# laprade117/interactive-unet

Hardware: AMD Instinct MI355X
Metric: voxels/sec (train step + full-volume predict) on 128^3 chunks (higher is better)
Workload: dtype bf16

## Files before the change

### include/iunet.h

```cpp
#ifndef IUNET_H
#define IUNET_H
#ifdef __cplusplus
extern "C" {
#endif

const char* iunet_last_error(void);
int iunet_abi_version(void);

long long iunet_pack_conv3_elems(int Cout, int Cin, int taps, int mode);
int iunet_pack_conv3(int dtype, const void* w, const void* scale, void* dst, int Cout, int Cin, int taps, int mode,
                     void* stream);
long long iunet_pack_first_conv_elems(int Cout, int Cin, int taps);
int iunet_pack_first_conv(int dtype, const void* w, const void* scale, void* dst, int Cout, int Cin, int taps,
                          void* stream);
int iunet_pack_convT(int dtype, const void* w, void* dst, int Cin, int Cout, int npos, void* stream);

int iunet_pack_desc_bytes(void);
int iunet_pack_batch(const void* descs, int n, int quant_max_cout, void* stream);

int iunet_conv3_fwd(int dtype, int nd, const void* x, long long x_sstride, void* y, long long y_sstride,
                    const void* wpk, const void* bias, void* stats, int N, int D, int H, int W, int Cin, int Cout,
                    int epi, int layout, void* stream);
int iunet_conv3_pick_layout(int nd, int N, int D, int H, int W, int Cin, int Cout);
int iunet_conv3_tile_pairs(int nd, int N, int D, int H, int W, int Cin, int Cout);
// ... 43 lines not shown
                            const void* weight, int tdtype, int kind, void* slab, void* out4, void* coef, int N, long long vox,
                            void* stream);
int iunet_f32_head_loss_bwd(const void* x, long long x_ss, int C0, const void* w, const void* bias, int ncls, const void* target,
                            const void* weight, int tdtype, const void* coef, void* dlogits, long long dl_ss, void* dx, long long dx_ss,
                            int N, long long vox, void* stream);
int iunet_f32_channel_sum(const void* t, long long t_ss, void* out, int C, int N, long long vox, void* stream);

int iunet_x2_convT_kc(int Cin);
int iunet_x2_prep(const void* w, void* wv, void* oscale, void* bias_out, const void* gamma, const void* beta, const void* mean,
                  const void* var, const void* bias_in, float eps, float act_in, float act_out, int Cout, int Cin, int taps,
                  int transposed, int chunk, void* stream);
int iunet_x2_prep_desc_bytes(void);
int iunet_x2_prep_batch(const void* table, int n, int rows, void* stream);
int iunet_x2m_prep_batch(const void* table, int n, int rows, void* stream);
int iunet_x2_first_conv_fwd(int nd, const void* x, int in_dtype, const long long* in_strides, void* y, long long y_sstride, int y_lo,
                            const void* w, const void* oscale, const void* bias, float act_scale, int N, int D, int H, int W, int Cin,
                            int Cout, int relu, void* stream);
int iunet_x2_pack_mode(int nd);
int iunet_x2_conv3_fwd(int nd, const void* x, long long x_sstride, int x_lo, void* y, long long y_sstride, int y_lo, const void* wpk,
                       const void* oscale, const void* bias, int N, int D, int H, int W, int Cin, int Cout, int epi, void* stream);
int iunet_x2_conv3_fwd_flag(int nd, const void* x, long long x_sstride, int x_lo, void* y, long long y_sstride, int y_lo, const void* wpk,
                            const void* oscale, const void* bias, int N, int D, int H, int W, int Cin, int Cout, int epi, void* sat, void* stream);
int iunet_x2_maxpool_fwd(int nd, const void* x, long long x_ss, int x_lo, void* y, long long y_ss, int y_lo, int C, int N, int Do,
                         int Ho, int Wo, void* stream);
int iunet_x2_convT_fwd(int nd, const void* x, long long x_ss, int x_lo, void* y, long long y_ss, int y_lo, const void* wpk,
                       const void* oscale, const void* bias, int N, int D, int H, int W, int Cin, int Cout, void* stream);
int iunet_x2_head_fwd(const void* x, long long x_ss, int x_lo, int C0, const void* w, const void* bias, float act_scale, int ncls,
                      void* logits, void* probs, void* cls, const long long* out_strides, float divisor, int accumulate, int N, int D,
                      int H, int W, void* stream);

long long iunet_x2m_w8_bytes(int Cout, int Cin);
int iunet_x2m_prep(const void* w, void* whi, void* w8, void* oscale, void* bias_out, const void* gamma, const void* beta, const void* mean,
                   const void* var, float eps, float act_in, float act_out, int Cout, int Cin, void* stream);
long long iunet_x2m_w8_bytes_nd(int nd, int Cout, int Cin);
int iunet_x2m_prep_nd(int nd, const void* w, void* whi, void* w8, void* oscale, void* bias_out, const void* gamma, const void* beta,
                      const void* mean, const void* var, float eps, float act_in, float act_out, int Cout, int Cin, void* stream);
int iunet_x2m_conv_fwd(int nd, const void* x, long long x_ss, const void* x8, long long x8_ss, void* y, long long y_ss, int y_lo, void* y8,
                       long long y8_ss, const void* w16, const void* w8, const void* oscale, const void* bias, int N, int D, int H, int W,
                       int Cin, int Cout, int epi, void* sat, void* stream);
int iunet_x2m_pool_fusable(int nd, int C);
int iunet_x2m_conv_pool_fwd(int nd, const void* x, long long x_ss, const void* x8, long long x8_ss, void* y, long long y_ss, int y_lo, void* y8,
                            long long y8_ss, void* py, long long py_ss, void* py8, long long py8_ss, const void* w16, const void* w8,
                            const void* oscale, const void* bias, int N, int D, int H, int W, int Cin, int Cout, int epi, void* sat, void* stream);
int iunet_x2m_first_stage_fusable(int nd, int cin, int c0, int N, int H, int W);
int iunet_x2m_first_stage_fwd(const void* x, int in_dtype, const long long* in_strides, const void* fw, const void* f_oscale, const void* f_bias,
                              float act_scale, void* y, long long y_ss, int y_lo, void* y8, long long y8_ss, void* py, long long py_ss, void* py8,
                              long long py8_ss, const void* w16, const void* w8, const void* oscale, const void* bias, int N, int H, int W,
                              void* sat, void* stream);
int iunet_x2m_head_fusable(int ncls, int C0);
int iunet_x2m_conv_head_fwd(int nd, const void* x, long long x_ss, const void* x8, long long x8_ss, const void* w16, const void* w8,
                            const void* oscale, const void* bias, const void* head_w, const void* head_b, float act_scale, int ncls,
                            void* logits, void* probs, void* cls, const long long* out_strides, float divisor, int accumulate, int N, int D,
                            int H, int W, int Cin, void* sat, void* stream);
int iunet_x2m_make8(const void* x, long long x_ss, int x_lo, void* x8, long long x8_ss, int C, int N, int D, int H, int W, void* stream);
int iunet_x2m_first_conv_fwd(int nd, const void* x, int in_dtype, const long long* in_strides, void* y, long long y_sstride, int y_lo,
                             void* y8, long long y8_sstride, const void* w, const void* oscale, const void* bias, float act_scale, int N,
                             int D, int H, int W, int Cin, int Cout, int relu, void* sat, void* stream);
int iunet_x2m_convT_fwd(int nd, const void* x, long long x_ss, int x_lo, void* y, long long y_ss, int y_lo, void* y8, long long y8_ss,
                        const void* wpk, const void* oscale, const void* bias, int N, int D, int H, int W, int Cin, int Cout, void* sat, void* stream);
int iunet_x2m_maxpool_fwd(int nd, const void* x, long long x_ss, const void* x8, long long x8_ss, void* y, long long y_ss, void* y8,
                          long long y8_ss, int C, int N, int Do, int Ho, int Wo, void* stream);
int iunet_x2m_conv3_fwd(const void* x, long long x_ss, const void* x8, long long x8_ss, void* y, long long y_ss, int y_lo, void* y8,
                        long long y8_ss, const void* w16, const void* w8, const void* oscale, const void* bias, int N, int D, int H, int W,
                        int Cin, int Cout, int epi, void* sat, void* stream);

typedef struct iunet_net iunet_net;
int iunet_net_create(int dim, int levels, int base, int cin, int ncls, int mode, float act_scale, iunet_net** out);
int iunet_net_create_ex(int dim, int levels, int base, int cin, int ncls, int mode, float act_scale, int norm, int groups, iunet_net** out);
int iunet_net_create_nested(int dim, int levels, int base, int cin, int ncls, int mode, iunet_net** out);
void iunet_net_destroy(iunet_net* net);
long long iunet_net_num_params(const iunet_net* net);
int iunet_net_num_tensors(const iunet_net* net);
int iunet_net_param(const iunet_net* net, int index, char* name, int name_cap, long long* offset, long long* numel);
long long iunet_net_packed_bytes(const iunet_net* net);
int iunet_net_load(iunet_net* net, const void* flat_params, void* packed, void* stream);
long long iunet_net_workspace_bytes(const iunet_net* net, int N, int D, int H, int W);
int iunet_net_forward(iunet_net* net, const void* x, int in_dtype, const long long* in_strides, int N, int D, int H, int W, void* workspace,
                      void* logits, void* probs, void* cls, const long long* out_strides, float divisor, int accumulate, void* stream);
int iunet_net_forward_argmax(iunet_net* net, const void* x_u8, void* cls_u8, int N, int D, int H, int W, void* workspace, void* stream);
long long iunet_net_eval_scratch_bytes(const iunet_net* net, int N, int D, int H, int W);
int iunet_net_eval_step(iunet_net* net, const void* x, int in_dtype, const long long* in_strides, const void* target, const void* weight,
                        int tdtype, int loss_kind, int N, int D, int H, int W, void* workspace, void* scratch, void* out4, void* stream);

int iunet_f8_pack_order(int taps, int Cin);
long long iunet_f8_pack_conv3_bytes(int Cout, int Cin, int taps);
int iunet_f8_pack_conv3(const void* w, const void* gamma, const void* beta, const void* mean, const void* var, float eps,
                        void* dst, void* wscale, void* bias_out, int Cout, int Cin, int taps, void* stream);
long long iunet_conv3_f8_workspace_elems(int nd, int N, int D, int H, int W, int Cin, int Cout);
int iunet_conv3_f8_fwd(int dtype, int nd, const void* x, long long x_sstride, void* y, long long y_sstride, const void* wpk,
                       const void* wscale, const void* bias, int N, int D, int H, int W, int Cin, int Cout, int epi,
                       void* workspace, void* stream);
int iunet_conv3_f8_fwd_q(int dtype, int nd, const void* x, long long x_sstride, int x_fmt, void* y, long long y_sstride, int y_fmt,
                         const void* wpk, const void* wscale, const void* bias, int N, int D, int H, int W, int Cin, int Cout, int epi,
                         void* workspace, void* stream);
int iunet_first_conv_fwd_q(int dtype, int nd, const void* x, int in_dtype, const long long* in_strides, void* y,
                           long long y_sstride_bytes, const void* w, const void* bias, int N, int D, int H, int W,
                           int Cin, int Cout, int relu, void* stream);
int iunet_maxpool_q_fwd(int nd, const void* x, long long x_ss_bytes, void* y, long long y_ss_bytes, int C, int N, int Do, int Ho, int Wo,
                        void* stream);
int iunet_convT_fwd_q(int dtype, int nd, const void* x, long long x_ss, void* y, long long y_ss_bytes, const void* wpk,
                      const void* bias, int N, int D, int H, int W, int Cin, int Cout, void* stream);

long long iunet_gn_precise_slab_bytes(int N, int C, long long vox);
int iunet_f32_gn_relu_fwd(const void* x, long long x_ss, void* y, long long y_ss, const void* gamma, const void* beta, int groups, float eps,
                          void* slab, void* scale, void* shift, int C, int N, long long vox, void* stream);
int iunet_x2_gn_relu_fwd(const void* x, long long x_ss, int x_lo, void* y, long long y_ss, int y_lo, const void* gamma, const void* beta,
// ... 202 lines not shown
```

### interactive-unet_amd/csrc/conv3_x2m.hip

```cpp
#include "common.h"
#include "x2_prep_desc.h"
#ifdef X2M_ABLATE_NO_MFMA
template <typename A, typename B> __device__ __forceinline__ f32x4 x2m_ablate(const A a, const B b, f32x4 c) {
  c[0] = fmaf(__builtin_bit_cast(float, (unsigned)__builtin_bit_cast(unsigned long long, *(const unsigned long long*)&a)),
              __builtin_bit_cast(float, (unsigned)__builtin_bit_cast(unsigned long long, *(const unsigned long long*)&b)), c[0]);
  return c;
}
#define X2M_MFMA16(a, b, c) x2m_ablate(a, b, c)
#define X2M_MFMA128(a, b, c) x2m_ablate(a, b, c)
#define X2M_MFMA32F8(a, b, c) x2m_ablate(a, b, c)
#else
#define X2M_MFMA16(a, b, c) __builtin_amdgcn_mfma_f32_16x16x32_f16(a, b, c, 0, 0, 0)
#define X2M_MFMA128(a, b, c) __builtin_amdgcn_mfma_scale_f32_16x16x128_f8f6f4(a, b, c, 0, 0, 0, 0, 0, 0)
#define X2M_MFMA32F8(a, b, c) __builtin_amdgcn_mfma_f32_16x16x32_fp8_fp8(a, b, c, 0, 0, 0)
#endif
#include <cstdlib>
#include <type_traits>

namespace {

typedef long i64;
typedef int i32x8 __attribute__((ext_vector_type(8)));
typedef u32x2_t u32x2;

// ... 33 lines not shown
  f16x8 hi;
#pragma unroll
  for (int c = 0; c < NCLS; ++c) l[c] = 0.f;
#pragma unroll
  for (int j = 0; j < 8; ++j) {
    const float v = fminf(fmaxf(r[j], -65504.f), 65504.f);
    const f16 h = (f16)v;
    const f16 lw = (f16)(v - (float)h);
    hi[j] = h;
    const float a = ((float)h + (float)lw) * p.inv_act;
#pragma unroll
    for (int c = 0; c < NCLS; ++c) l[c] = fmaf(a, hw[c * 32 + q * 8 + j], l[c]);
  }
  if (ok && p.sat != nullptr) x2_note_saturation(p.sat, hi);
#pragma unroll
  for (int c = 0; c < NCLS; ++c) {
    l[c] = __fadd_rn(l[c], __shfl_xor(l[c], 16));
    l[c] = __fadd_rn(l[c], __shfl_xor(l[c], 32));
    l[c] = __fadd_rn(l[c], hw[NCLS * 32 + c]);
  }
}
template <int NCLS>
__device__ __forceinline__ void x2m_head_store(const ConvX2MParams& p, const float (&l)[NCLS], bool ok, int n_img, long long nvox, long long vo,
                                               int gz, int gy, int gx) {
  if (!ok) return;
  const long long obase = n_img * p.oN + gz * p.oD + gy * p.oH + gx * p.oW;
  float mx = l[0];
#pragma unroll
  for (int c = 1; c < NCLS; ++c) mx = fmaxf(mx, l[c]);
  if (p.logits) {
#pragma unroll
    for (int c = 0; c < NCLS; ++c) p.logits[obase + c * p.oC] = l[c];
  }
  float e[NCLS], sum = 0.f;
#pragma unroll
  for (int c = 0; c < NCLS; ++c) { e[c] = expf(l[c] - mx); sum += e[c]; }
  float pr[NCLS];
  pr[0] = __fdiv_rn(e[0], sum);
  float pm = pr[0]; int am = 0;
#pragma unroll
  for (int c = 1; c < NCLS; ++c) { pr[c] = __fdiv_rn(e[c], sum); if (pr[c] > pm) { pm = pr[c]; am = c; } }
  if (p.cls) p.cls[n_img * nvox + vo] = (unsigned char)am;
  if (p.probs) {
#pragma unroll
    for (int c = 0; c < NCLS; ++c) {
      float* o = p.probs + obase + c * p.oC;
      float rr = p.accumulate ? __fadd_rn(*o, pr[c]) : pr[c];
      if (p.divisor != 1.0f) rr = __fdiv_rn(rr, p.divisor);
      *o = rr;
    }
  }
}

template <bool SMALL, int HEAD = 0, bool POOL = false>
__global__ __launch_bounds__((XMTile<SMALL>::NCW * 64 + XM_NLT), 1) void conv3_x2m_kernel(ConvX2MParams p) {
  static_assert(!(POOL && HEAD > 0), "the pooled conv is an encoder conv: no head");
  using TL = XMTile<SMALL>;
  constexpr int NCW = TL::NCW, NLT = XM_NLT, NLW = NLT / 64;
  constexpr int TZ = TL::TZ, TY = TL::TY, TX = TL::TX;
  constexpr int NI = TZ * TY / NCW, NR = NI;
  constexpr int PZ = TZ + 2, PY = TY + 2, PX = TX + 2;
  constexpr int NPIX = PZ * PY * PX;
  constexpr int PLANE16 = ((NPIX * 16 + 255) / 256) * 256;
  constexpr int A16 = 2 * PLANE16;
  constexpr int NCMB = 5, W16 = NCMB * 3 * 2 * 1024;
  constexpr int ZS = 192;
  constexpr int PLANE8 = PZ * ZS * 16;
  constexpr int A8 = 2 * PLANE8;
  constexpr int W128 = 2 * 3 * 2 * 2 * 1024, W32 = 3 * 2 * 512, W8 = W128 + W32;
  constexpr int OFF_A16 = 0, OFF_W16 = A16, OFF_A8 = OFF_W16 + W16, OFF_W8 = OFF_A8 + A8, OFF_E = OFF_W8 + W8;
  constexpr int OFF_P = OFF_E + 256;
  static_assert(NI == 4 && NCW * NI == TZ * TY, "a consumer wave owns 4 rows of one z slice");

  extern __shared__ __attribute__((aligned(256))) unsigned char smem[];

  const int tid = threadIdx.x, lane = tid & 63;
  const int wave = __builtin_amdgcn_readfirstlane(tid >> 6);
  const int cob = blockIdx.y;
  const int nbricks = p.N * p.nbz * p.nby * p.nbx;
  const int xcd = (blockIdx.x + (nbricks < 8 ? blockIdx.y : 0)) & 7, slot = blockIdx.x >> 3;
  const int sx = slot % p.bx, sy = (slot / p.bx) % p.by, sz = slot / (p.bx * p.by);
  const int b_begin = (int)((long long)xcd * nbricks / 8), b_end = (int)((long long)(xcd + 1) * nbricks / 8);
  const int nchunk = p.Cin / 16;
  const int npairs = (b_end - b_begin) * nchunk;
  if (npairs <= 0) return;
  const long long plane_stride = (long long)p.D * p.H * p.W * 8;
  const long long plane16b = (long long)p.D * p.H * p.W * 16;

  auto tile_origin = [&](int k, int& n_img, int& z0, int& y0, int& x0) -> bool {
    int b = b_begin + k;
    const int Bx = b % p.nbx; b /= p.nbx;
    const int By = b % p.nby; b /= p.nby;
    const int Bz = b % p.nbz; n_img = b / p.nbz;
    const int tz = Bz * p.bz + sz, ty = By * p.by + sy, tx = Bx * p.bx + sx;
    z0 = tz * TZ; y0 = ty * TY; x0 = tx * TX;
    return tz < p.tilesZ && ty < p.tilesY && tx < p.tilesX;
  };
  const unsigned lds0 = (unsigned)(size_t)(__attribute__((address_space(3))) unsigned char*)smem;
  if (tid < 64) ((float*)(smem + OFF_E))[tid] = tid < 32 ? p.oscale[cob * 32 + tid] : (p.epi != 0 ? p.bias[cob * 32 + tid - 32] : 0.f);
  if constexpr (HEAD > 0) {
    for (int i = tid; i < HEAD * 33; i += (int)blockDim.x) ((float*)(smem + OFF_E + 256))[i] = i < HEAD * 32 ? p.head_w[i] : p.head_b[i - HEAD * 32];
  }

  if (wave >= NCW) {
    const unsigned* zero16 = iunet_opaque_ptr((const unsigned*)g_xm_zero16);
    const int lt = tid - NCW * 64;
    const int lw = __builtin_amdgcn_readfirstlane(lt >> 6);
    auto dma_piece = [&](const unsigned char* gsrc, unsigned dst) {
      unsigned keep;
      asm volatile("s_mov_b32 %0, m0\n\ts_mov_b32 m0, %2\n\ts_nop 0\n\tglobal_load_lds_dwordx4 %1, off\n\ts_mov_b32 m0, %0"
                   : "=&s"(keep) : "v"(gsrc), "s"(dst) : "memory");
    };
    auto dma_weights = [&](const unsigned char* ws, int off, int bytes) {
      const int npiece = bytes / 1024;
      for (int piece = lw; piece < npiece; piece += NLW)
        dma_piece(ws + piece * 1024 + (lt & 63) * 16, __builtin_amdgcn_readfirstlane(lds0 + off + piece * 1024));
    };
    constexpr int AIT = (PLANE16 / 16 + NLT - 1) / NLT;
    int pcoord[AIT];
#pragma unroll
    for (int it = 0; it < AIT; ++it) {
      const int pix = min(lt + it * NLT, NPIX - 1);
      const int px = pix % PX, t2 = pix / PX;
      pcoord[it] = px | ((t2 % PY) << 8) | ((t2 / PY) << 16);
    }
    constexpr int NSLOT = PZ * ZS;
    constexpr int DIT = (NSLOT + NLT - 1) / NLT;
    static_assert(NSLOT % 64 == 0, "an e4m3 plane is whole wave instructions");
    int dcoord[DIT];
#pragma unroll
    for (int it = 0; it < DIT; ++it) {
      const int s = lt + it * NLT;
      const int pz = s / ZS, rem = s - pz * ZS, py = rem / PX, px = rem - py * PX;
      dcoord[it] = (s < NSLOT && rem < PY * PX) ? (px | (py << 8) | (pz << 16)) : -1;
    }
    auto dma16 = [&](int k) {
      const int tile = k / nchunk, chunk = k - tile * nchunk;
      int n_img, z0, y0, x0;
      tile_origin(tile, n_img, z0, y0, x0);
      dma_weights((const unsigned char*)p.w16 + ((long long)cob * nchunk + chunk) * W16, OFF_W16, W16);
      const f16* xc = (const f16*)p.x + (long long)n_img * p.x_sstride + (long long)chunk * 2 * plane_stride;
#pragma unroll
      for (int it = 0; it < AIT; ++it) {
        const int base = it * NLT + lw * 64;
        if (base < PLANE16 / 16) {
          const int pix = lt + it * NLT;
          const int px = pcoord[it] & 255, py = (pcoord[it] >> 8) & 255, pz = pcoord[it] >> 16;
          const int gz = z0 + pz - 1, gy = y0 + py - 1, gx = x0 + px - 1;
          const bool ok = pix < NPIX && (unsigned)gz < (unsigned)p.D && (unsigned)gy < (unsigned)p.H && (unsigned)gx < (unsigned)p.W;
          const long long goff = (((long long)gz * p.H + gy) * p.W + gx) * 8;
          if (pix < PLANE16 / 16) {
#pragma unroll
            for (int e = 0; e < 2; ++e)
              dma_piece(ok ? (const unsigned char*)(xc + e * plane_stride + goff) : (const unsigned char*)zero16,
                        __builtin_amdgcn_readfirstlane(lds0 + OFF_A16 + e * PLANE16 + base * 16));
          }
        }
      }
    };
    auto dma8 = [&](int k) {
      const int tile = k / nchunk, chunk = k - tile * nchunk;
      int n_img, z0, y0, x0;
      tile_origin(tile, n_img, z0, y0, x0);
      dma_weights((const unsigned char*)p.w8 + ((long long)cob * nchunk + chunk) * W8, OFF_W8, W8);
      const unsigned char* xc = (const unsigned char*)p.x8 + (long long)n_img * p.x8_sstride + (long long)chunk * plane16b;
#pragma unroll
      for (int it = 0; it < DIT; ++it) {
        const int base = it * NLT + lw * 64;
        if (base < NSLOT) {
          const int c = dcoord[it];
          const int gz = z0 + (c >> 16) - 1, gy = y0 + ((c >> 8) & 255) - 1, gx = x0 + (c & 255) - 1;
          const bool ok = c >= 0 && (unsigned)gz < (unsigned)p.D && (unsigned)gy < (unsigned)p.H && (unsigned)gx < (unsigned)p.W;
          const long long goff = (((long long)gz * p.H + gy) * p.W + gx) * 16;
          dma_piece(ok ? xc + goff : (const unsigned char*)zero16, __builtin_amdgcn_readfirstlane(lds0 + OFF_A8 + base * 16));
        }
      }
    };
    auto make_hi8 = [&]() {
      f16x8 va[DIT], vb[DIT];
#pragma unroll
      for (int it = 0; it < DIT; ++it) {
        const int c = dcoord[it];
        const int pix = c >= 0 ? ((c >> 16) * PY + ((c >> 8) & 255)) * PX + (c & 255) : 0;
        va[it] = *(const f16x8*)(smem + OFF_A16 + pix * 16);
        vb[it] = *(const f16x8*)(smem + OFF_A16 + PLANE16 + pix * 16);
      }
#pragma unroll
      for (int it = 0; it < DIT; ++it) {
        const int s = lt + it * NLT;
        if (s < NSLOT) {
          const u32x2 a = x2m_hi8(va[it]), b = x2m_hi8(vb[it]);
          *(u32x4*)(smem + OFF_A8 + PLANE8 + s * 16) = dcoord[it] >= 0 ? u32x4{a[0], a[1], b[0], b[1]} : u32x4{0u, 0u, 0u, 0u};
        }
      }
    };
#ifdef X2M_ABLATE_NO_WAIT
    auto landed = [&]() {};
#else
    auto landed = [&]() { asm volatile("s_waitcnt vmcnt(0)" ::: "memory"); };
#endif
    [[maybe_unused]] f16x8 pw_hi; [[maybe_unused]] u32x2 pw_lo8;
    [[maybe_unused]] f16* pw_dst = nullptr; [[maybe_unused]] unsigned char* pw_dst8 = nullptr; [[maybe_unused]] long long pw_plane = 0;
    [[maybe_unused]] auto pool_words = [&](int tile) {
      pw_dst = nullptr;
      if (lt >= NCW * 32) return;
      const int q = lt & 3, x8 = (lt >> 2) & 7, py = (lt >> 5) & 3, pz = lt >> 7;
      const unsigned char* a = smem + OFF_P + (((((4 * pz + (py >> 1)) * 2 + (py & 1)) * 8 + x8) * 4 + q) * 32);
      const unsigned char* b = a + 2 * (2 * 8 * 4 * 32);
      const u32x4 a0 = *(const u32x4*)a, a1 = *(const u32x4*)(a + 16), b0 = *(const u32x4*)b, b1 = *(const u32x4*)(b + 16);
      unsigned kk[8];
#pragma unroll
      for (int j = 0; j < 4; ++j) { kk[j] = max(a0[j], b0[j]); kk[4 + j] = max(a1[j], b1[j]); }
      int n_img, z0, y0, x0;
      tile_origin(tile, n_img, z0, y0, x0);
      const int Do = p.D >> 1, Ho = p.H >> 1, Wo = p.W >> 1;
      const int oz = (z0 >> 1) + pz, oy = (y0 >> 1) + py, ox = (x0 >> 1) + x8;
      if (oz < Do && oy < Ho && ox < Wo) {
        const long long onvox = (long long)Do * Ho * Wo, ovo = ((long long)oz * Ho + oy) * Wo + ox;
        x2m_pool_unkeys(kk, pw_hi, pw_lo8);
        pw_dst = (f16*)p.pool_y + (long long)n_img * p.pool_y_ss + ((long long)(cob * 4 + q) * onvox + ovo) * 8;
        pw_dst8 = (unsigned char*)p.pool_y8 + (long long)n_img * p.pool_y8_ss + x2m_off(cob * 4 + q, ovo, onvox);
        pw_plane = onvox * 16;
      }
    };
    [[maybe_unused]] auto pool_store = [&]() {
      if (pw_dst != nullptr) {
        *(f16x8*)pw_dst = pw_hi;
        *(u32x2*)pw_dst8 = pw_lo8;
      }
    };
    dma16(0);
    landed();
    lds_barrier();
    for (int k = 0; k < npairs; ++k) {
#ifndef X2M_ABLATE_NO_COPIES
      dma8(k);
#endif
#if !defined(X2M_ABLATE_NO_HI8) && !defined(X2M_ABLATE_NO_COPIES)
      make_hi8();
#endif
      landed();
      lds_barrier();
#ifndef X2M_ABLATE_NO_COPIES
      if (k + 1 < npairs) dma16(k + 1);
#endif
      const bool pool_now = POOL && k > 0 && k % nchunk == 0;
      if constexpr (POOL) { if (pool_now) pool_words(k / nchunk - 1); }
      landed();
      if constexpr (POOL) { if (pool_now) pool_store(); }
      lds_barrier();
    }
    if constexpr (POOL) {
      lds_barrier();
      pool_words(npairs / nchunk - 1);
      pool_store();
    }
    return;
  }

  const int l15 = lane & 15, q = lane >> 4;
  const int row_first = wave * NI;
  int col_off[NCMB];
#pragma unroll
  for (int c = 0; c < NCMB; ++c) {
    const int col = min(2 * c + (q >> 1), 8);
    col_off[c] = ((col / 3) * PY * PX + (col % 3)) * 16;
  }
  const int rbase16 = (q & 1) * PLANE16 + ((((row_first / TY) * PY + (row_first % TY)) * PX) + l15) * 16;
  int coff[2];
#pragma unroll
  for (int g = 0; g < 2; ++g) {
    const int col = q == 0 ? f8k_col(g, 0) : q == 1 ? f8k_col(g, 1) : q == 2 ? f8k_col(g, 2) : f8k_col(g, 3);
    coff[g] = ((col / 3) * ZS + (col % 3)) * 16;
  }
  const int coff8 = (2 * ZS + 2) * 16 + (q >> 1) * PLANE8 + (q & 1) * 8;
  const int rbase8 = (((row_first / TY) * ZS + (row_first % TY) * PX) + l15) * 16;

  f32x4 acc[2][NI];
#pragma unroll
  for (int m = 0; m < 2; ++m)
#pragma unroll
    for (int n = 0; n < NI; ++n) acc[m][n] = f32x4{0.f, 0.f, 0.f, 0.f};

  using I0 = std::integral_constant<int, 0>; using I1 = std::integral_constant<int, 1>; using I2 = std::integral_constant<int, 2>;
  using I3 = std::integral_constant<int, 3>; using I4 = std::integral_constant<int, 4>; using I5 = std::integral_constant<int, 5>;
  using I6 = std::integral_constant<int, 6>; using I7 = std::integral_constant<int, 7>; using I8 = std::integral_constant<int, 8>;

  f16x8 R16[2][NR + 2], A16f[2][3][2];
  i32x8 R8f[2][NR + 2], A8f[2][2];
  i64 R8n[NR + 2], A8n[3][2];

  auto load_group = [&](int c, auto BUF) {
    constexpr int b = decltype(BUF)::value;
    const unsigned char* ab = smem + OFF_A16 + rbase16;
    const unsigned char* wl = smem + OFF_W16 + lane * 16;
#pragma unroll
    for (int r = 0; r < NR + 2; ++r) R16[b][r] = *(const f16x8*)(ab + r * PX * 16 + col_off[c]);
#pragma unroll
    for (int dy = 0; dy < 3; ++dy) {
      A16f[b][dy][0] = *(const f16x8*)(wl + ((c * 3 + dy) * 2 + 0) * 1024);
      A16f[b][dy][1] = *(const f16x8*)(wl + ((c * 3 + dy) * 2 + 1) * 1024);
    }
  };
  auto group_mfmas = [&](auto BUF, bool reads_pending) {
    constexpr int b = decltype(BUF)::value;
#pragma unroll
    for (int dy = 0; dy < 3; ++dy)
#pragma unroll
      for (int n = 0; n < NI; ++n) {
        acc[0][n] = X2M_MFMA16(A16f[b][dy][0], R16[b][n + dy], acc[0][n]);
        acc[1][n] = X2M_MFMA16(A16f[b][dy][1], R16[b][n + dy], acc[1][n]);
      }
    if (reads_pending) {
      constexpr int NRD = NR + 2 + 6, MPR = (3 * NI * 2) / NRD;
#pragma unroll
      for (int i = 0; i < NRD; ++i) {
        __builtin_amdgcn_sched_group_barrier(0x100, 1, 0);
        __builtin_amdgcn_sched_group_barrier(0x008, MPR, 0);
      }
    }
    __builtin_amdgcn_sched_barrier(0);
  };

  auto rd128 = [&](const unsigned char* ptr, int second) -> i32x8 {
    const u32x4 lo = *(const u32x4*)ptr, hi = *(const u32x4*)(ptr + second);
    return i32x8{(int)lo[0], (int)lo[1], (int)lo[2], (int)lo[3], (int)hi[0], (int)hi[1], (int)hi[2], (int)hi[3]};
  };
  auto load_sub = [&](auto SG) {
    constexpr int sg = decltype(SG)::value, g = sg / 3, dy = sg % 3;
    const unsigned char* ab = smem + OFF_A8;
    const unsigned char* wl = smem + OFF_W8;
    if constexpr (g < 2) {
#pragma unroll
      for (int m = 0; m < 2; ++m) A8f[sg & 1][m] = rd128(wl + ((g * 3 + dy) * 2 + m) * 2048 + lane * 16, 1024);
      constexpr int r0 = dy == 0 ? 0 : NR - 1 + dy, r1 = dy == 0 ? NR : NR + dy;
#pragma unroll
      for (int r = r0; r < r1; ++r) R8f[g][r] = rd128(ab + rbase8 + coff[g] + r * PX * 16, PLANE8);
    } else if constexpr (dy == 0) {
#pragma unroll
      for (int d = 0; d < 3; ++d)
#pragma unroll
        for (int m = 0; m < 2; ++m) A8n[d][m] = *(const i64*)(wl + W128 + (d * 2 + m) * 512 + lane * 8);
#pragma unroll
      for (int r = 0; r < NR + 2; ++r) R8n[r] = *(const i64*)(ab + rbase8 + coff8 + r * PX * 16);
    }
  };
  auto mfma_sub = [&](auto SG, auto NREADS) {
// ... 32 lines not shown
    {
      const f32x4* ep = (const f32x4*)(smem + OFF_E) + 2 * q;
      const f32x4 w0 = ep[0], w1 = ep[1], b0 = ep[8], b1 = ep[9];
#pragma unroll
      for (int j = 0; j < 4; ++j) { os_r[j] = w0[j]; os_r[4 + j] = w1[j]; bias_r[j] = b0[j]; bias_r[4 + j] = b1[j]; }
    }
    const float relu_floor = p.epi == 2 ? 0.f : -65504.f;
    [[maybe_unused]] float hl[HEAD > 0 ? HEAD : 1];
    [[maybe_unused]] unsigned pool_k[8];
#pragma unroll
    for (int n = 0; n < NI; ++n) {
      const int row = row_first + n;
      const int gz = z0 + row / TY, gy = y0 + row % TY, gx = x0 + l15;
      const bool ok = gz < p.D && gy < p.H && gx < p.W;
      const long long vo = ((long long)gz * p.H + gy) * p.W + gx;
      float r[8];
#pragma unroll
      for (int j = 0; j < 8; ++j) {
        r[j] = fmaf(j < 4 ? acc[0][n][j] : acc[1][n][j - 4], os_r[j], bias_r[j]);
        if constexpr (HEAD > 0) { if (p.epi == 2) r[j] = fmaxf(r[j], 0.f); }
        else r[j] = __builtin_amdgcn_fmed3f(r[j], relu_floor, 65504.f);
      }
      if constexpr (HEAD > 0) {
        float lf[HEAD];
        x2m_head_logits<HEAD>(p, (const float*)(smem + OFF_E + 256), r, q, ok, lf);
#pragma unroll
        for (int c = 0; c < HEAD; ++c) hl[c] = q == n ? lf[c] : hl[c];
      } else {
      f16x8 hi, lo;
      u32x2 lo8, hi8;
      x2m_split8<true>(r, hi, lo, lo8, hi8);
      if (ok) {
        *(f16x8*)(yout + (long long)(cob * 4 + q) * plane_stride + vo * 8) = hi;
        if (p.y_lo >= 0) *(f16x8*)(yout + (long long)(p.y_lo + cob * 4 + q) * plane_stride + vo * 8) = lo;
        if (p.y8 != nullptr) {
          unsigned char* y8 = (unsigned char*)p.y8 + (long long)n_img * p.y8_sstride + x2m_off(cob * 4 + q, vo, plane16b / 16);
          *(u32x2*)y8 = lo8;
        }
        if (p.sat != nullptr) x2_note_saturation(p.sat, hi);
      }
      if constexpr (POOL) {
        unsigned kk[8];
        x2m_pool_keys(hi, lo8, kk);
        if ((n & 1) == 0) {
#pragma unroll
          for (int j = 0; j < 8; ++j) pool_k[j] = kk[j];
        } else {
#pragma unroll
          for (int j = 0; j < 8; ++j) {
            kk[j] = max(kk[j], pool_k[j]);
            kk[j] = max(kk[j], lane_xor1(kk[j]));
          }
          if (!(l15 & 1)) {
            unsigned char* dst = smem + OFF_P + ((((wave * 2 + (n >> 1)) * 8 + (l15 >> 1)) * 4 + q) * 32);
            *(u32x4*)dst = u32x4{kk[0], kk[1], kk[2], kk[3]};
            *(u32x4*)(dst + 16) = u32x4{kk[4], kk[5], kk[6], kk[7]};
          }
        }
      }
      }
      acc[0][n] = f32x4{0.f, 0.f, 0.f, 0.f};
      acc[1][n] = f32x4{0.f, 0.f, 0.f, 0.f};
    }
    if constexpr (HEAD > 0) {
      const int row = row_first + q;
      const int gz = z0 + row / TY, gy = y0 + row % TY, gx = x0 + l15;
      x2m_head_store<HEAD>(p, hl, gz < p.D && gy < p.H && gx < p.W, n_img, plane16b / 16, ((long long)gz * p.H + gy) * p.W + gx, gz, gy, gx);
    }
  };

  lds_barrier();
  load_group(0, I0{});
  __builtin_amdgcn_sched_barrier(0);
  for (int k = 0; k < npairs; ++k) {
    load_group(1, I1{}); group_mfmas(I0{}, true);
    load_group(2, I0{}); group_mfmas(I1{}, true);
    load_group(3, I1{}); group_mfmas(I0{}, true);
    load_group(4, I0{}); group_mfmas(I1{}, true);
    lds_barrier();
    load_sub(I0{});
    group_mfmas(I0{}, true);
    load_sub(I1{}); mfma_sub(I0{}, N6{});
    load_sub(I2{}); mfma_sub(I1{}, N6{});
    load_sub(I3{}); mfma_sub(I2{}, N12{});
    load_sub(I4{}); mfma_sub(I3{}, N6{});
    load_sub(I5{}); mfma_sub(I4{}, N6{});
    load_sub(I6{}); mfma_sub(I5{}, N12{});
    lds_barrier();
    load_group(0, I0{});
    mfma_sub(I6{}, N4{}); mfma_sub(I7{}, N4{}); mfma_sub(I8{}, N4{});
    const int tile = k / nchunk;
    if (k - tile * nchunk == nchunk - 1) tile_epilogue(tile);
  }
  if constexpr (POOL) lds_barrier();
}


constexpr int X2M2_W8 = 4 * 2 * 2 * 1024 + 2 * 2 * 512;
__host__ __device__ inline int x2m2_w8_offset(int tap, int m, int b, int e, int o, int row) {
  if (tap == 8) return 4 * 2 * 2 * 1024 + ((b * 2 + m) * 64 + (2 * e + o) * 16 + row) * 8;
  const int G = b * 2 + (tap >> 2), q = tap & 3;
  return (((G * 2 + m) * 2 + e) * 64 + q * 16 + row) * 16 + 8 * o;
}

template <int HEAD = 0, bool POOL = false, bool FIRST = false>
__global__ __launch_bounds__(8 * 64 + XM_NLT, 1) void conv2_x2m_kernel(ConvX2MParams p) {
  static_assert(!(POOL && HEAD > 0), "the pooled conv is an encoder conv: no head");
  static_assert(!(FIRST && HEAD > 0), "the first stage's second conv has no head");
  constexpr int NCW = 8, NLT = XM_NLT, NLW = NLT / 64;
  constexpr int TY = 16, TX = 32, FX = 2, NI = 4, NR = 2;
  constexpr int PY = TY + 2, PX = TX + 2, NPIX = PY * PX;
  constexpr int PLANE = ((NPIX * 16 + 255) / 256) * 256;
  constexpr int A16 = 4 * PLANE, W16 = 3 * 3 * 2 * 1024;
  constexpr int A8 = 4 * PLANE, W128 = 4 * 2 * 2 * 1024, W8 = X2M2_W8;
  constexpr int OFF_A16 = 0, OFF_W16 = A16, OFF_A8 = OFF_W16 + W16, OFF_W8 = OFF_A8 + A8, OFF_E = OFF_W8 + W8;
  constexpr int OFF_P = OFF_E + 256;
  constexpr int FPX = PX + 2, FPIX = 7 * FPX, FPATCH = 3 * FPIX * 2;
  constexpr int OFF_F = OFF_P + (POOL ? 8 * 16 * 4 * 32 : 0);

  extern __shared__ __attribute__((aligned(256))) unsigned char smem[];
  const int tid = threadIdx.x, lane = tid & 63;
  const int wave = __builtin_amdgcn_readfirstlane(tid >> 6);
  const int cob = blockIdx.y;
  const int nbricks = p.N * p.nby * p.nbx;
// ... 450 lines not shown
      }
      }
      acc[0][n] = f32x4{0.f, 0.f, 0.f, 0.f};
      acc[1][n] = f32x4{0.f, 0.f, 0.f, 0.f};
    }
    if constexpr (HEAD > 0) {
      const int gy = y0 + row_first + q / FX, gx = x0 + (q % FX) * 16 + l15;
      x2m_head_store<HEAD>(p, hl, gy < p.H && gx < p.W, n_img, nvox, (long long)gy * p.W + gx, 0, gy, gx);
    }
  };

  lds_barrier();
  load_group(0, I0{});
  __builtin_amdgcn_sched_barrier(0);
  for (int k = 0; k < npairs; ++k) {
    load_group(1, I1{}); group_mfmas(I0{});
    load_group(2, I0{}); group_mfmas(I1{});
    lds_barrier();
    load_g8(0, I0{});
    group_mfmas(I0{});
    load_g8(1, I1{}); mfma_g8(I0{});
    load_g8(2, I0{}); mfma_g8(I1{});
    load_g8(3, I1{}); mfma_g8(I0{});
    load_tap8(); mfma_g8(I1{});
    lds_barrier();
    load_group(0, I0{});
    mfma_tap8();
    const int tile = k / nchunk;
    if (k - tile * nchunk == nchunk - 1) tile_epilogue(tile);
  }
  if constexpr (POOL) lds_barrier();
}

template <int HEAD, bool POOL = false, bool FIRST = false>
int launch_x2m_2d(ConvX2MParams p, hipStream_t stream) {
  constexpr int PLANE = ((18 * 34 * 16 + 255) / 256) * 256;
  const int lds = 8 * PLANE + 18432 + X2M2_W8 + 256 + (HEAD > 0 ? 2048 : 0) + (POOL ? 8 * 16 * 4 * 32 : 0) + (FIRST ? 4 * 3 * 7 * 36 * 2 + 4 * 256 : 0);
  IUNET_SET_MAX_LDS((conv2_x2m_kernel<HEAD, POOL, FIRST>), lds);
  p.tilesZ = 1; p.tilesY = (p.H + 15) / 16; p.tilesX = (p.W + 31) / 32;
  const int ncob = p.Cout / 32;
  iunet_brick_shape(2, ncob, 1, p.tilesY, p.tilesX, &p.bz, &p.by, &p.bx);
  p.nbz = 1; p.nby = (p.tilesY + p.by - 1) / p.by; p.nbx = (p.tilesX + p.bx - 1) / p.bx;
  const long long nbricks = (long long)p.N * p.nby * p.nbx;
  const int table = 8 * (ncob == 1 ? 32 : ncob == 2 ? 16 : ncob <= 4 ? 8 : 4);
  int groups = table / 8 / (p.by * p.bx);
  while (groups > 1 && nbricks / 8 < groups) groups >>= 1;
  if (groups < 1) groups = 1;
  const int gx = 8 * p.by * p.bx * groups;
  hipLaunchKernelGGL((conv2_x2m_kernel<HEAD, POOL, FIRST>), dim3(gx, ncob), dim3(8 * 64 + XM_NLT), lds, stream, p);
  IUNET_CHECK_HIP(hipGetLastError());
  return IUNET_OK;
}

template <bool SMALL, int HEAD = 0, bool POOL = false>
int launch_x2m(ConvX2MParams p, hipStream_t stream) {
  using TL = XMTile<SMALL>;
  constexpr int PZ = TL::TZ + 2, NPIX = PZ * 10 * 18;
  constexpr int PLANE16 = ((NPIX * 16 + 255) / 256) * 256, PLANE8 = PZ * 192 * 16;
  const int lds = 2 * PLANE16 + 30720 + 2 * PLANE8 + F8K_WSTEP + 256 + (HEAD > 0 ? 2048 : 0) + (POOL ? TL::NCW * 64 * 32 : 0);
  IUNET_SET_MAX_LDS((conv3_x2m_kernel<SMALL, HEAD, POOL>), lds);
  p.tilesZ = (p.D + TL::TZ - 1) / TL::TZ; p.tilesY = (p.H + TL::TY - 1) / TL::TY; p.tilesX = (p.W + TL::TX - 1) / TL::TX;
  const int ncob = p.Cout / 32;
  iunet_brick_shape(3, ncob, p.tilesZ, p.tilesY, p.tilesX, &p.bz, &p.by, &p.bx);
  p.nbz = (p.tilesZ + p.bz - 1) / p.bz; p.nby = (p.tilesY + p.by - 1) / p.by; p.nbx = (p.tilesX + p.bx - 1) / p.bx;
  const int gx = 8 * p.bz * p.by * p.bx;
  hipLaunchKernelGGL((conv3_x2m_kernel<SMALL, HEAD, POOL>), dim3(gx, ncob), dim3(TL::NCW * 64 + XM_NLT), lds, stream, p);
  IUNET_CHECK_HIP(hipGetLastError());
  return IUNET_OK;
}

__device__ __forceinline__ unsigned xm_e4m3(float v) {
  const int a = __builtin_amdgcn_cvt_pk_fp8_f32(__builtin_amdgcn_fmed3f(v, -448.0f, 448.0f), 0.f, 0, false);
  return (unsigned)a & 0xffu;
}
__device__ __forceinline__ void x2m_prep_row(const float* __restrict__ w, float* __restrict__ whi, unsigned char* __restrict__ w8,
                                             float* __restrict__ oscale, float* __restrict__ bias_out,
                                             const float* __restrict__ gamma, const float* __restrict__ beta,
                                             const float* __restrict__ mean, const float* __restrict__ var, float eps,
                                             float act_in, float act_out, int Cout, int Cin, int taps, int co, float* red) {
#pragma clang fp contract(off)
  const int tid = threadIdx.x;
  float a = 1.0f;
  if (gamma) { const float s = var[co] + eps; a = gamma[co] / sqrtf(s); }
  const int n = Cin * taps;
  const float* wc = w + (long long)co * n;
  float m = 0.f;
  for (int i = tid; i < n; i += 256) m = fmaxf(m, fabsf(gamma ? wc[i] * a : wc[i]));
  red[tid] = m;
  __syncthreads();
  for (int o = 128; o > 0; o >>= 1) { if (tid < o) red[tid] = fmaxf(red[tid], red[tid + o]); __syncthreads(); }
  m = red[0];
  float s = 1.0f;
  if (m > 0.f && m < INFINITY) {
    int e;
    (void)frexpf(m, &e);
    int k = 10 - e;
    k = k < -40 ? -40 : k > 40 ? 40 : k;
    s = ldexpf(1.0f, k);
  }
  const int cob = co >> 5, r32 = co & 31;
  const int mt = (r32 >> 2) & 1, row = (r32 >> 3) * 4 + (r32 & 3);
  const int nchunk = Cin >> 4;
  for (int i = tid; i < (Cin >> 3) * taps; i += 256) {
    const int g8 = i / taps, tap = i - g8 * taps;
    const int chunk = g8 >> 1, o = g8 & 1;
    const int dz = tap / 9, dy = (tap / 3) % 3, dx = tap % 3, col = dz * 3 + dx;
    unsigned long long ph = 0, pl = 0;
#pragma unroll
    for (int j = 0; j < 8; ++j) {
      const int ci = g8 * 8 + j;
      const float v0 = wc[(long long)ci * taps + tap];
      float v = (gamma ? v0 * a : v0) * s;
      v = fminf(fmaxf(v, -65504.f), 65504.f);
      const f16 h = (f16)v;
      const float res = v - (float)h;
      whi[(long long)co * n + (long long)ci * taps + tap] = (float)h;
      ph |= (unsigned long long)xm_e4m3((float)h * 0.0625f) << (8 * j);
      pl |= (unsigned long long)xm_e4m3(res * 256.0f) << (8 * j);
    }
// ... 119 lines not shown
  IUNET_REQUIRE(Cout > 0 && Cout % 32 == 0 && Cin > 0 && Cin % 32 == 0, "x2m_prep: channels must be positive multiples of 32 (%d, %d)", Cout, Cin);
  IUNET_REQUIRE(!gamma || (beta && mean && var), "x2m_prep: a BatchNorm fold needs gamma, beta, mean and var");
  int e1, e2;
  IUNET_REQUIRE(act_in > 0.f && act_out > 0.f && frexpf(act_in, &e1) == 0.5f && frexpf(act_out, &e2) == 0.5f,
                "x2m_prep: the activation scales must be powers of two (got %g, %g)", act_in, act_out);
  hipLaunchKernelGGL(x2m_prep_kernel, dim3(Cout), dim3(256), 0, (hipStream_t)stream, (const float*)w, (float*)whi, (unsigned char*)w8,
                     (float*)oscale, (float*)bias_out, (const float*)gamma, (const float*)beta, (const float*)mean, (const float*)var,
                     eps, act_in, act_out, Cout, Cin, nd == 3 ? 27 : 9);
  IUNET_CHECK_HIP(hipGetLastError());
  return IUNET_OK;
}

int iunet_x2m_prep_batch(const void* table, int n, int rows, void* stream) {
  IUNET_REQUIRE(table != nullptr && n > 0 && rows > 0, "x2m_prep_batch: empty table");
  hipLaunchKernelGGL(x2m_prep_batch_kernel, dim3(rows), dim3(256), 0, (hipStream_t)stream, (const X2PrepDesc*)table, n);
  IUNET_CHECK_HIP(hipGetLastError());
  return IUNET_OK;
}

int iunet_x2m_make8(const void* x, long long x_ss, int x_lo, void* x8, long long x8_ss, int C, int N, int D, int H, int W, void* stream) {
  IUNET_REQUIRE(x && x8, "x2m_make8: null pointer");
  IUNET_REQUIRE(C > 0 && C % 16 == 0, "x2m_make8: C must be a multiple of 16 (got %d)", C);
  IUNET_REQUIRE_GRID("x2m_make8", N, D, H, W);
  const long long vox = (long long)D * H * W;
  dim3 grid((unsigned)((vox + 255) / 256), C / 16, N);
  hipLaunchKernelGGL(x2m_make8_kernel, grid, dim3(256), 0, (hipStream_t)stream, (const f16*)x, x_ss, x_lo, (unsigned char*)x8, x8_ss, C / 16, vox);
  IUNET_CHECK_HIP(hipGetLastError());
  return IUNET_OK;
}

int iunet_x2m_maxpool_fwd(int nd, const void* x, long long x_ss, const void* x8, long long x8_ss, void* y, long long y_ss, void* y8,
                          long long y8_ss, int C, int N, int Do, int Ho, int Wo, void* stream) {
  IUNET_REQUIRE(x && x8 && y && y8, "x2m_maxpool: null pointer");
  IUNET_REQUIRE(nd == 2 || nd == 3, "x2m_maxpool: nd must be 2 or 3");
  IUNET_REQUIRE(C > 0 && C % 16 == 0 && N > 0 && Do > 0 && Ho > 0 && Wo > 0, "x2m_maxpool: bad shape");
  const long long total = (long long)Do * Ho * Wo * (C / 16);
  dim3 grid((unsigned)((total + 255) / 256), N);
  if (nd == 3) hipLaunchKernelGGL((x2m_maxpool_kernel<3>), grid, dim3(256), 0, (hipStream_t)stream, (const f16*)x, x_ss, (const unsigned char*)x8, x8_ss,
                                  (f16*)y, y_ss, (unsigned char*)y8, y8_ss, C / 16, Do, Ho, Wo);
  else hipLaunchKernelGGL((x2m_maxpool_kernel<2>), grid, dim3(256), 0, (hipStream_t)stream, (const f16*)x, x_ss, (const unsigned char*)x8, x8_ss,
                          (f16*)y, y_ss, (unsigned char*)y8, y8_ss, C / 16, Do, Ho, Wo);
  IUNET_CHECK_HIP(hipGetLastError());
  return IUNET_OK;
}

int iunet_x2m_conv_fwd(int nd, const void* x, long long x_ss, const void* x8, long long x8_ss, void* y, long long y_ss, int y_lo, void* y8,
                       long long y8_ss, const void* w16, const void* w8, const void* oscale, const void* bias, int N, int D, int H, int W,
                       int Cin, int Cout, int epi, void* sat, void* stream);
int iunet_x2m_conv3_fwd(const void* x, long long x_ss, const void* x8, long long x8_ss, void* y, long long y_ss, int y_lo, void* y8,
                        long long y8_ss, const void* w16, const void* w8, const void* oscale, const void* bias, int N, int D, int H, int W,
                        int Cin, int Cout, int epi, void* sat, void* stream) {
  return iunet_x2m_conv_fwd(3, x, x_ss, x8, x8_ss, y, y_ss, y_lo, y8, y8_ss, w16, w8, oscale, bias, N, D, H, W, Cin, Cout, epi, sat, stream);
}
static int x2m_conv_impl(const char* who, int nd, const void* x, long long x_ss, const void* x8, long long x8_ss, void* y, long long y_ss, int y_lo,
                         void* y8, long long y8_ss, void* py, long long py_ss, void* py8, long long py8_ss, const void* w16, const void* w8,
                         const void* oscale, const void* bias, int N, int D, int H, int W, int Cin, int Cout, int epi, void* sat, void* stream) {
  IUNET_REQUIRE(nd == 2 || nd == 3, "%s: nd must be 2 or 3", who);
  IUNET_REQUIRE(nd == 3 || D == 1, "%s: 2-D needs D == 1", who);
  IUNET_REQUIRE(x && x8 && y && w16 && w8 && oscale, "%s: null pointer", who);
  IUNET_REQUIRE(N > 0 && D > 0 && H > 0 && W > 0, "%s: bad shape N %d, %d x %d x %d", who, N, D, H, W);
  IUNET_REQUIRE(Cin >= 32 && Cout >= 32 && Cin % 32 == 0 && Cout % 32 == 0, "%s: channels must be positive multiples of 32 (%d -> %d)", who, Cin, Cout);
  IUNET_REQUIRE(epi >= 0 && epi <= 2, "%s: bad epilogue %d", who, epi);
  IUNET_REQUIRE(epi == 0 || bias != nullptr, "%s: epilogue %d needs a bias", who, epi);
  const bool pool = py != nullptr;
  if (pool) {
    IUNET_REQUIRE(py8 != nullptr, "%s: the pooled tensor needs its m8 planes", who);
    IUNET_REQUIRE(H % 2 == 0 && W % 2 == 0 && (nd == 2 || D % 2 == 0), "%s: the pooled grid needs even sizes (%d, %d, %d)", who, D, H, W);
  }
  ConvX2MParams p;
  p.x = x; p.x_sstride = x_ss; p.x8 = x8; p.x8_sstride = x8_ss; p.y = y; p.y_sstride = y_ss; p.y_lo = y_lo; p.y8 = y8; p.y8_sstride = y8_ss;
  p.w16 = w16; p.w8 = w8; p.oscale = (const float*)oscale; p.bias = (const float*)bias;
  p.N = N; p.D = D; p.H = H; p.W = W; p.Cin = Cin; p.Cout = Cout; p.epi = epi; p.sat = (int*)sat;
  p.tilesZ = p.tilesY = p.tilesX = 0;
  p.bz = p.by = p.bx = p.nbz = p.nby = p.nbx = 0;
  p.head_w = p.head_b = nullptr; p.inv_act = 0.f; p.logits = p.probs = nullptr; p.cls = nullptr;
  p.oN = p.oC = p.oD = p.oH = p.oW = 0; p.divisor = 1.f; p.accumulate = 0;
  p.pool_y = py; p.pool_y_ss = py_ss; p.pool_y8 = py8; p.pool_y8_ss = py8_ss;
  p.f_x = p.f_w = nullptr; p.f_oscale = p.f_bias = nullptr; p.f_sN = p.f_sH = p.f_sW = 0; p.f_dtype = 0; p.f_act = 0.f;
  hipStream_t s = (hipStream_t)stream;
  if (nd == 2) return pool ? launch_x2m_2d<0, true>(p, s) : launch_x2m_2d<0>(p, s);
  const long long big_tiles = (long long)N * ((D + 3) / 4) * ((H + 7) / 8) * ((W + 15) / 16);
  const bool small = big_tiles * (Cout / 32) < 128;
  if (pool) return small ? launch_x2m<true, 0, true>(p, s) : launch_x2m<false, 0, true>(p, s);
  return small ? launch_x2m<true>(p, s) : launch_x2m<false>(p, s);
}

int iunet_x2m_conv_fwd(int nd, const void* x, long long x_ss, const void* x8, long long x8_ss, void* y, long long y_ss, int y_lo, void* y8,
                       long long y8_ss, const void* w16, const void* w8, const void* oscale, const void* bias, int N, int D, int H, int W,
                       int Cin, int Cout, int epi, void* sat, void* stream) {
  return x2m_conv_impl("x2m_conv3", nd, x, x_ss, x8, x8_ss, y, y_ss, y_lo, y8, y8_ss, nullptr, 0, nullptr, 0, w16, w8, oscale, bias, N, D, H, W,
                       Cin, Cout, epi, sat, stream);
}

int iunet_x2m_pool_fusable(int nd, int C) {
  static const int mode = getenv("IUNET_X2M_POOL") ? atoi(getenv("IUNET_X2M_POOL")) : 1;
  if (mode == 0 || (nd != 2 && nd != 3)) return 0;
  if (nd == 3) return 1;
  return mode == 3 ? 0 : mode == 4 ? C != 64 : 1;
}

int iunet_x2m_conv_pool_fwd(int nd, const void* x, long long x_ss, const void* x8, long long x8_ss, void* y, long long y_ss, int y_lo, void* y8,
                            long long y8_ss, void* py, long long py_ss, void* py8, long long py8_ss, const void* w16, const void* w8,
                            const void* oscale, const void* bias, int N, int D, int H, int W, int Cin, int Cout, int epi, void* sat, void* stream) {
  IUNET_REQUIRE(py && py8, "x2m_conv_pool: null pooled tensor");
  return x2m_conv_impl("x2m_conv_pool", nd, x, x_ss, x8, x8_ss, y, y_ss, y_lo, y8, y8_ss, py, py_ss, py8, py8_ss, w16, w8, oscale, bias, N, D, H, W,
                       Cin, Cout, epi, sat, stream);
}

int iunet_x2m_first_stage_fusable(int nd, int cin, int c0, int N, int H, int W) {
  static const int mode = getenv("IUNET_X2M_FIRST") ? atoi(getenv("IUNET_X2M_FIRST")) : 1;
  if (mode == 0 || nd != 2 || cin != 1 || c0 != 32 || N < 1 || H < 1 || W < 1) return 0;
  if (mode >= 2) return 1;
  return !iunet_x2m_pool_fusable(nd, c0) && (long long)N * ((H + 15) / 16) * ((W + 31) / 32) >= 2048;
}

int iunet_x2m_first_stage_fwd(const void* x, int in_dtype, const long long* in_strides, const void* fw, const void* f_oscale, const void* f_bias,
                              float act_scale, void* y, long long y_ss, int y_lo, void* y8, long long y8_ss, void* py, long long py_ss, void* py8,
                              long long py8_ss, const void* w16, const void* w8, const void* oscale, const void* bias, int N, int H, int W,
                              void* sat, void* stream) {
  IUNET_REQUIRE(x && in_strides && fw && f_oscale && f_bias && y && w16 && w8 && oscale && bias, "x2m_first_stage: null pointer");
  IUNET_REQUIRE(in_dtype >= 0 && in_dtype <= 3, "x2m_first_stage: bad input dtype %d", in_dtype);
  IUNET_REQUIRE(N > 0 && H > 0 && W > 0, "x2m_first_stage: bad shape N %d, %d x %d", N, H, W);
  IUNET_REQUIRE((py == nullptr) == (py8 == nullptr), "x2m_first_stage: the pooled tensor is hi planes AND m8 planes");
  IUNET_REQUIRE(py == nullptr || (H % 2 == 0 && W % 2 == 0), "x2m_first_stage: the pooled grid needs even sizes (%d, %d)", H, W);
  int e1;
  IUNET_REQUIRE(act_scale > 0.f && frexpf(act_scale, &e1) == 0.5f, "x2m_first_stage: the activation scale must be a power of two (got %g)", act_scale);
  ConvX2MParams p;
  p.x = nullptr; p.x_sstride = 0; p.x8 = nullptr; p.x8_sstride = 0; p.y = y; p.y_sstride = y_ss; p.y_lo = y_lo; p.y8 = y8; p.y8_sstride = y8_ss;
  p.w16 = w16; p.w8 = w8; p.oscale = (const float*)oscale; p.bias = (const float*)bias;
  p.N = N; p.D = 1; p.H = H; p.W = W; p.Cin = 32; p.Cout = 32; p.epi = 2; p.sat = (int*)sat;
  p.tilesZ = p.tilesY = p.tilesX = 0;
  p.bz = p.by = p.bx = p.nbz = p.nby = p.nbx = 0;
  p.head_w = p.head_b = nullptr; p.inv_act = 0.f; p.logits = p.probs = nullptr; p.cls = nullptr;
  p.oN = p.oC = p.oD = p.oH = p.oW = 0; p.divisor = 1.f; p.accumulate = 0;
  p.pool_y = py; p.pool_y_ss = py_ss; p.pool_y8 = py8; p.pool_y8_ss = py8_ss;
  p.f_x = x; p.f_sN = in_strides[0]; p.f_sH = in_strides[3]; p.f_sW = in_strides[4]; p.f_dtype = in_dtype;
  p.f_w = fw; p.f_oscale = (const float*)f_oscale; p.f_bias = (const float*)f_bias; p.f_act = act_scale;
  hipStream_t s = (hipStream_t)stream;
  return py != nullptr ? launch_x2m_2d<0, true, true>(p, s) : launch_x2m_2d<0, false, true>(p, s);
}

int iunet_x2m_head_fusable(int ncls, int C0) {
  static const int off = getenv("IUNET_X2M_HEAD") ? (atoi(getenv("IUNET_X2M_HEAD")) == 0) : 0;
  return !off && ncls >= 2 && ncls <= 3 && C0 == 32;
}

int iunet_x2m_conv_head_fwd(int nd, const void* x, long long x_ss, const void* x8, long long x8_ss, const void* w16, const void* w8,
                            const void* oscale, const void* bias, const void* head_w, const void* head_b, float act_scale, int ncls,
                            void* logits, void* probs, void* cls, const long long* out_strides, float divisor, int accumulate, int N, int D,
                            int H, int W, int Cin, void* sat, void* stream) {
  IUNET_REQUIRE(nd == 2 || nd == 3, "x2m_conv_head: nd must be 2 or 3");
  IUNET_REQUIRE(nd == 3 || D == 1, "x2m_conv_head: 2-D needs D == 1");
  IUNET_REQUIRE(x && x8 && w16 && w8 && oscale && bias && head_w && head_b && out_strides, "x2m_conv_head: null pointer");
  IUNET_REQUIRE_GRID("x2m_conv_head", N, D, H, W);
  IUNET_REQUIRE(Cin >= 32 && Cin % 32 == 0, "x2m_conv_head: Cin must be a positive multiple of 32 (got %d)", Cin);
  IUNET_REQUIRE(ncls == 2 || ncls == 3, "x2m_conv_head: 2 or 3 classes (got %d)", ncls);
  int e1;
  IUNET_REQUIRE(act_scale > 0.f && frexpf(act_scale, &e1) == 0.5f, "x2m_conv_head: the activation scale must be a power of two (got %g)", act_scale);
  ConvX2MParams p;
  p.x = x; p.x_sstride = x_ss; p.x8 = x8; p.x8_sstride = x8_ss; p.y = nullptr; p.y_sstride = 0; p.y_lo = -1; p.y8 = nullptr; p.y8_sstride = 0;
  p.w16 = w16; p.w8 = w8; p.oscale = (const float*)oscale; p.bias = (const float*)bias;
  p.N = N; p.D = D; p.H = H; p.W = W; p.Cin = Cin; p.Cout = 32; p.epi = 2; p.sat = (int*)sat;
  p.tilesZ = p.tilesY = p.tilesX = 0;
  p.bz = p.by = p.bx = p.nbz = p.nby = p.nbx = 0;
  p.head_w = (const float*)head_w; p.head_b = (const float*)head_b; p.inv_act = 1.0f / act_scale;
  p.logits = (float*)logits; p.probs = (float*)probs; p.cls = (unsigned char*)cls;
  p.oN = out_strides[0]; p.oC = out_strides[1]; p.oD = out_strides[2]; p.oH = out_strides[3]; p.oW = out_strides[4];
  p.divisor = divisor; p.accumulate = accumulate;
  p.pool_y = p.pool_y8 = nullptr; p.pool_y_ss = p.pool_y8_ss = 0;
  p.f_x = p.f_w = nullptr; p.f_oscale = p.f_bias = nullptr; p.f_sN = p.f_sH = p.f_sW = 0; p.f_dtype = 0; p.f_act = 0.f;
  hipStream_t s = (hipStream_t)stream;
  if (nd == 2) return ncls == 2 ? launch_x2m_2d<2>(p, s) : launch_x2m_2d<3>(p, s);
  const long long big_tiles = (long long)N * ((D + 3) / 4) * ((H + 7) / 8) * ((W + 15) / 16);
  if (big_tiles < 128)
    return ncls == 2 ? launch_x2m<true, 2>(p, s) : launch_x2m<true, 3>(p, s);
  return ncls == 2 ? launch_x2m<false, 2>(p, s) : launch_x2m<false, 3>(p, s);
}

}
```

### interactive-unet_amd/csrc/net.hip

```cpp
#include "common.h"
#include <algorithm>
#include <cstdio>
#include <cstdlib>
#include <cstring>
#include <string>
#include <vector>

extern "C" {
int iunet_x2_prep(const void*, void*, void*, void*, const void*, const void*, const void*, const void*, const void*, float, float, float,
                  int, int, int, int, int, void*);
int iunet_x2_first_conv_fwd(int, const void*, int, const long long*, void*, long long, int, const void*, const void*, const void*, float,
                            int, int, int, int, int, int, int, void*);
int iunet_x2_conv3_fwd(int, const void*, long long, int, void*, long long, int, const void*, const void*, const void*, int, int, int, int,
                       int, int, int, void*);
int iunet_x2_maxpool_fwd(int, const void*, long long, int, void*, long long, int, int, int, int, int, int, void*);
int iunet_x2_convT_fwd(int, const void*, long long, int, void*, long long, int, const void*, const void*, const void*, int, int, int, int,
                       int, int, void*);
int iunet_x2_head_fwd(const void*, long long, int, int, const void*, const void*, float, int, void*, void*, void*, const long long*, float,
                      int, int, int, int, int, void*);
int iunet_x2m_prep_nd(int, const void*, void*, void*, void*, void*, const void*, const void*, const void*, const void*, float, float, float, int, int, void*);
int iunet_x2m_conv_fwd(int, const void*, long long, const void*, long long, void*, long long, int, void*, long long, const void*, const void*,
                       const void*, const void*, int, int, int, int, int, int, int, void*, void*);
long long iunet_x2m_w8_bytes_nd(int, int, int);
int iunet_x2m_head_fusable(int, int);
int iunet_x2m_conv_head_fwd(int, const void*, long long, const void*, long long, const void*, const void*, const void*, const void*, const void*,
                            const void*, float, int, void*, void*, void*, const long long*, float, int, int, int, int, int, int, void*, void*);
int iunet_x2m_first_conv_fwd(int, const void*, int, const long long*, void*, long long, int, void*, long long, const void*, const void*, const void*,
                             float, int, int, int, int, int, int, int, void*, void*);
int iunet_x2m_convT_fwd(int, const void*, long long, int, void*, long long, int, void*, long long, const void*, const void*, const void*, int, int,
                        int, int, int, int, void*, void*);
int iunet_x2_conv3_fwd_flag(int, const void*, long long, int, void*, long long, int, const void*, const void*, const void*, int, int, int, int,
                            int, int, int, void*, void*);
int iunet_x2m_maxpool_fwd(int, const void*, long long, const void*, long long, void*, long long, void*, long long, int, int, int, int, int, void*);
int iunet_x2m_pool_fusable(int, int);
int iunet_x2m_first_stage_fusable(int, int, int, int, int, int);
int iunet_x2m_first_stage_fwd(const void*, int, const long long*, const void*, const void*, const void*, float, void*, long long, int, void*, long long, void*,
                              long long, void*, long long, const void*, const void*, const void*, const void*, int, int, int, void*, void*);
int iunet_x2m_conv_pool_fwd(int, const void*, long long, const void*, long long, void*, long long, int, void*, long long, void*, long long, void*, long long,
                            const void*, const void*, const void*, const void*, int, int, int, int, int, int, int, void*, void*);
int iunet_x2m_conv3_fwd(const void*, long long, const void*, long long, void*, long long, int, void*, long long, const void*, const void*,
                        const void*, const void*, int, int, int, int, int, int, int, void*, void*);
long long iunet_x2m_w8_bytes(int, int);
int iunet_pack_conv3(int, const void*, const void*, void*, int, int, int, int, void*);
int iunet_pack_first_conv(int, const void*, const void*, void*, int, int, int, void*);
int iunet_pack_convT(int, const void*, void*, int, int, int, void*);
long long iunet_pack_conv3_elems(int, int, int, int);
long long iunet_pack_first_conv_elems(int, int, int);
int iunet_conv3_pick_layout(int, int, int, int, int, int, int);
int iunet_x2_pack_mode(int);
int iunet_conv3_compact_ok(int, int, int, int, int, int, int, int, int);
int iunet_first_conv_fwd(int, int, const void*, int, const long long*, void*, long long, const void*, const void*, void*, int, int, int,
                         int, int, int, int, void*);
int iunet_conv3_fwd(int, int, const void*, long long, void*, long long, const void*, const void*, void*, int, int, int, int, int, int,
                    int, int, void*);
int iunet_maxpool_fwd(int, int, const void*, long long, void*, long long, int, int, int, int, int, void*);
int iunet_convT_fwd(int, int, const void*, long long, void*, long long, const void*, const void*, int, int, int, int, int, int, void*);
long long iunet_gn_precise_slab_bytes(int, int, long long);
int iunet_x2_gn_relu_fwd(const void*, long long, int, void*, long long, int, const void*, const void*, int, float, float, void*, void*, void*, int, int,
                         long long, void*, void*);
int iunet_head_loss_num_parts(int, long long);
int iunet_head_loss_fwd(int, const void*, long long, int, const void*, const void*, int, const void*, const void*, int, int, void*, void*,
                        void*, int, long long, void*);
int iunet_head_fwd(int, const void*, long long, int, const void*, const void*, int, void*, void*, void*, const long long*, float, int, int,
                   int, int, int, void*);
}

namespace {

__global__ void net_fold_bn_kernel(const float* __restrict__ gamma, const float* __restrict__ beta, const float* __restrict__ mean,
                                   const float* __restrict__ var, float eps, float* __restrict__ scale, float* __restrict__ bias, int C) {
#pragma clang fp contract(off)
  const int c = blockIdx.x * blockDim.x + threadIdx.x;
  if (c >= C) return;
  const float s = var[c] + eps;
  const float a = gamma[c] / sqrtf(s);
  const float t = mean[c] * a;
  scale[c] = a;
  bias[c] = beta[c] - t;
}

long long align256(long long v) { return (v + 255) & ~255ll; }

struct Param { std::string name; long long off, numel; };

struct ConvOp {
  int ci, co, first;
  long long w, bn;
  long long pk[4];
  long long aux;
};
struct UpOp { int ci, co; long long w, b, pk, aux; };

}

struct iunet_net {
  int dim, levels, base, cin, ncls, mode;
  int norm = 0, groups = 8;
  float act_scale;
  int taps, npos;
  std::vector<int> ch;
  std::vector<Param> params;
  long long nparams = 0;
  std::vector<ConvOp> conv;
  std::vector<UpOp> up;
  bool nested = false;
  std::vector<std::pair<int, int>> nodes;
  long long head_w = 0, head_b = 0;
  long long packed_bytes = 0, scratch_off = 0;
  const float* flat = nullptr;
  unsigned char* packed = nullptr;
};

namespace {

int stage_index(const iunet_net* n, bool dec, int l) { return dec ? n->levels + (n->levels - 2 - l) : l; }

struct WsLayout { std::vector<long long> a, b, cat, pin, am, catm, pinm; long long raw = -1, gnslab = -1, gnsc = -1, gnsh = -1; long long bytes; };

WsLayout ws_layout(const iunet_net* n, int N, int D, int H, int W) {
  WsLayout L;
  const int lv = n->levels, mul = n->mode == 2 ? 2 : 1;
  long long off = n->mode >= 2 ? 256 : 0;
  auto take = [&](long long elems) { const long long o = off; off = align256(off + elems * 2); return o; };
  L.a.resize(lv); L.b.resize(lv); L.cat.resize(lv, -1); L.pin.resize(lv, -1);
  L.am.resize(lv, -1); L.catm.resize(lv, -1); L.pinm.resize(lv, -1);
  if (n->nested) {
    for (int l = 0; l < lv; ++l) {
      const long long v = (long long)(n->dim == 3 ? D >> l : 1) * (H >> l) * (W >> l);
      L.cat[l] = take((long long)N * (lv - l) * n->ch[l] * v);
      L.a[l] = take((long long)N * n->ch[l] * v);
      L.b[l] = -1;
      if (l > 0) L.pin[l] = take((long long)N * n->ch[l - 1] * v);
    }
    L.b[0] = take((long long)N * n->ch[0] * (n->dim == 3 ? D : 1) * H * W);
    L.bytes = off;
    return L;
  }
  if (n->mode == 3) {
    for (int l = 0; l < lv; ++l) {
      const long long v = (long long)(n->dim == 3 ? D >> l : 1) * (H >> l) * (W >> l);
      L.a[l] = take((long long)N * n->ch[l] * v); L.am[l] = take((long long)N * n->ch[l] * v / 2);
      L.b[l] = take((long long)N * 2 * n->ch[l] * v);
      if (l < lv - 1) { L.cat[l] = take((long long)N * 2 * n->ch[l] * v); L.catm[l] = take((long long)N * n->ch[l] * v); }
      if (l > 0) { L.pin[l] = take((long long)N * n->ch[l - 1] * v); L.pinm[l] = take((long long)N * n->ch[l - 1] * v / 2); }
    }
    L.bytes = off;
    return L;
  }
  for (int l = 0; l < lv; ++l) {
// ... 68 lines not shown
    dims(i + 1, di, hi, wi);
    const long long v = vox(i), vi = vox(i + 1);
    const int c = n->ch[i], cn = n->ch[i + 1];
    const long long cat_ss = (long long)(lv - i) * c * v;
    unsigned char* up = WS + L.cat[i] + (long long)j * c * v * 2;
    const UpOp& u = n->up[k];
    rc = iunet_convT_fwd(mode, dim, WS + L.cat[i + 1] + (long long)(j - 1) * cn * vi * 2, (long long)(lv - i - 1) * cn * vi, up, cat_ss, K + u.pk,
                         n->flat + u.b, N, di, hi, wi, cn, c, stream);
    if (rc) return rc;
    const ConvOp& c1 = n->conv[2 * (lv + k)];
    const ConvOp& c2 = n->conv[2 * (lv + k) + 1];
    rc = conv16(n, c1, WS + L.cat[i], cat_ss, WS + L.a[i], (long long)c * v, N, d, h, w, stream);
    if (rc) return rc;
    const bool last = k + 1 == n->nodes.size();
    rc = conv16(n, c2, WS + L.a[i], (long long)c * v, last ? WS + L.b[0] : up, last ? (long long)c * v : cat_ss, N, d, h, w, stream);
    if (rc) return rc;
  }
  if (!logits && !probs && !cls) return IUNET_OK;
  const long long v0 = vox(0);
  const long long dflt[5] = {n->ncls * v0, v0, (long long)H * W, W, 1};
  const int c0 = n->ch[0];
  return iunet_head_fwd(mode, WS + L.b[0], (long long)c0 * v0, c0, n->flat + n->head_w, n->flat + n->head_b, n->ncls, logits, probs, cls,
                        out_strides ? out_strides : dflt, divisor, accumulate, N, D, H, W, stream);
}

}

extern "C" {

int iunet_net_create_ex(int dim, int levels, int base, int cin, int ncls, int mode, float act_scale, int norm, int groups, iunet_net** out);
int iunet_net_create(int dim, int levels, int base, int cin, int ncls, int mode, float act_scale, iunet_net** out) {
  return iunet_net_create_ex(dim, levels, base, cin, ncls, mode, act_scale, 0, 8, out);
}
static int net_create(int dim, int levels, int base, int cin, int ncls, int mode, float act_scale, int norm, int groups, bool nested, iunet_net** out);
int iunet_net_create_ex(int dim, int levels, int base, int cin, int ncls, int mode, float act_scale, int norm, int groups, iunet_net** out) {
  return net_create(dim, levels, base, cin, ncls, mode, act_scale, norm, groups, false, out);
}
int iunet_net_create_nested(int dim, int levels, int base, int cin, int ncls, int mode, iunet_net** out) {
  IUNET_REQUIRE(mode == 0 || mode == 1, "net_create_nested: mode must be 0 (fp16) or 1 (bf16), got %d", mode);
  return net_create(dim, levels, base, cin, ncls, mode, 0.f, 0, 8, true, out);
}
static int net_create(int dim, int levels, int base, int cin, int ncls, int mode, float act_scale, int norm, int groups, bool nested, iunet_net** out) {
  IUNET_REQUIRE(out != nullptr, "net_create: null handle pointer");
  IUNET_REQUIRE(norm == 0 || norm == 1, "net_create: norm must be 0 (batch) or 1 (group), got %d", norm);
  IUNET_REQUIRE(norm == 0 || (mode == 2 && groups > 0 && base % groups == 0), "net_create: GroupNorm runs in mode 2 (fp16x2) with groups dividing base (mode %d, %d groups)", mode, groups);
  IUNET_REQUIRE(dim == 2 || dim == 3, "net_create: dim must be 2 or 3 (got %d)", dim);
  if (nested) IUNET_REQUIRE(levels >= 2 && levels <= 9, "net_create_nested: levels must be 2..9 (got %d)", levels);
  else IUNET_REQUIRE(levels >= 2 && levels <= 6, "net_create: levels must be 2..6 (got %d)", levels);
  IUNET_REQUIRE(base > 0 && base % 32 == 0, "net_create: base channels must be a positive multiple of 32 (got %d)", base);
  IUNET_REQUIRE(cin >= 1 && cin <= 4, "net_create: 1..4 input channels (got %d)", cin);
  IUNET_REQUIRE(ncls >= 2 && ncls <= 10, "net_create: 2..10 classes (app.py:162; got %d)", ncls);
  IUNET_REQUIRE(mode >= 0 && mode <= 3, "net_create: mode must be 0 (fp16), 1 (bf16), 2 (fp16x2) or 3 (fp16x2, cross terms on fp8), got %d", mode);
  iunet_net* n = new iunet_net();
  n->dim = dim; n->levels = levels; n->base = base; n->cin = cin; n->ncls = ncls; n->mode = mode;
  n->norm = norm; n->groups = groups;
  n->act_scale = act_scale > 0.f ? act_scale : 64.0f;
  n->taps = dim == 3 ? 27 : 9; n->npos = dim == 3 ? 8 : 4;
  for (int l = 0; l < levels; ++l) n->ch.push_back(base << l);
  long long off = 0, pk = 0;
  auto add = [&](const std::string& name, long long numel) { n->params.push_back({name, off, numel}); const long long o = off; off += numel; return o; };
  auto pk_take = [&](long long bytes) { const long long o = pk; pk = align256(pk + bytes); return o; };
  long long max_virtual = 0;
  auto stage = [&](const std::string& prefix, int ci, int co) {
    for (int j = 1; j <= 2; ++j) {
      ConvOp op;
      op.ci = j == 1 ? ci : co; op.co = co; op.first = (prefix == "enc0" && j == 1);
      const std::string c = prefix + ".conv" + std::to_string(j), b = prefix + ".bn" + std::to_string(j);
      op.w = add(c + ".weight", (long long)co * op.ci * n->taps);
      op.bn = add(b + ".weight", co); add(b + ".bias", co); add(b + ".running_mean", co); add(b + ".running_var", co);
      for (int k = 0; k < 4; ++k) op.pk[k] = -1;
      const int vci = (mode == 2 || (mode == 3 && op.first)) ? 3 * op.ci : op.ci;
      if (op.first) op.pk[1] = pk_take(iunet_pack_first_conv_elems(co, vci, n->taps) * 2);
      else if (mode == 3) {
        op.pk[1] = pk_take(iunet_pack_conv3_elems(co, op.ci, n->taps, dim == 3 ? 2 : 6) * 2);
        op.pk[0] = pk_take(iunet_x2m_w8_bytes_nd(dim, co, op.ci));
      } else {
        op.pk[1] = pk_take(iunet_pack_conv3_elems(co, vci, n->taps, mode == 2 ? iunet_x2_pack_mode(dim) : 2) * 2);
        if (mode != 2) {
          const bool compact2d = n->taps == 9 && iunet_conv3_compact_ok(2, 1, 1, 16, 32, op.ci, co, 0, 0);
          if (co % 64 == 0 && n->taps == 9 && op.ci > 64 && !compact2d) op.pk[0] = pk_take(iunet_pack_conv3_elems(co, op.ci, n->taps, 0) * 2);
          const char* nc = getenv("IUNET_NO_COMPACT");
          if (((n->taps == 27 && op.ci > 32) || compact2d) && !(nc && nc[0])) op.pk[3] = pk_take(iunet_pack_conv3_elems(co, op.ci, n->taps, 6) * 2);
        }
      }
      op.aux = pk_take(2ll * co * 4);
      if (mode >= 2 && 3ll * co * op.ci * n->taps > max_virtual) max_virtual = 3ll * co * op.ci * n->taps;
      n->conv.push_back(op);
    }
  };
  for (int l = 0; l < levels; ++l) stage("enc" + std::to_string(l), l == 0 ? cin : n->ch[l - 1], n->ch[l]);
  n->nested = nested;
  for (int j = 1; j < levels && nested; ++j)
    for (int i = 0; i + j < levels; ++i) {
      n->nodes.push_back({i, j});
      UpOp u;
      u.ci = n->ch[i + 1]; u.co = n->ch[i];
      const std::string p = "dec" + std::to_string(i) + "_" + std::to_string(j);
      u.w = add(p + ".up.weight", (long long)u.ci * u.co * n->npos);
      u.b = add(p + ".up.bias", u.co);
      u.pk = pk_take((long long)u.ci * u.co * n->npos * 2);
      u.aux = pk_take(2ll * u.co * 4);
      n->up.push_back(u);
      stage(p, (j + 1) * n->ch[i], n->ch[i]);
    }
  for (int l = levels - 2; l >= 0 && !nested; --l) {
    UpOp u;
    u.ci = n->ch[l + 1]; u.co = n->ch[l];
    const std::string p = "dec" + std::to_string(l);
    u.w = add(p + ".up.weight", (long long)u.ci * u.co * n->npos);
    u.b = add(p + ".up.bias", u.co);
    u.pk = pk_take((long long)(mode >= 2 ? 2 : 1) * u.ci * u.co * n->npos * 2);
    u.aux = pk_take(2ll * u.co * 4);
    if (mode >= 2 && 2ll * u.ci * u.co * n->npos > max_virtual) max_virtual = 2ll * u.ci * u.co * n->npos;
    n->up.push_back(u);
    stage(p, 2 * n->ch[l], n->ch[l]);
  }
  n->head_w = add("head.weight", (long long)ncls * n->ch[0]);
  n->head_b = add("head.bias", ncls);
  n->nparams = off;
  n->scratch_off = pk;
  n->packed_bytes = pk + max_virtual * 4;
  *out = n;
  return IUNET_OK;
}

void iunet_net_destroy(iunet_net* n) { delete n; }

long long iunet_net_num_params(const iunet_net* n) { return n ? n->nparams : 0; }
int iunet_net_num_tensors(const iunet_net* n) { return n ? (int)n->params.size() : 0; }

int iunet_net_param(const iunet_net* n, int index, char* name, int name_cap, long long* offset, long long* numel) {
  IUNET_REQUIRE(n != nullptr, "net_param: null handle");
  IUNET_REQUIRE(index >= 0 && index < (int)n->params.size(), "net_param: index %d out of range", index);
  const Param& p = n->params[index];
  if (name && name_cap > 0) snprintf(name, name_cap, "%s", p.name.c_str());
  if (offset) *offset = p.off;
  if (numel) *numel = p.numel;
  return IUNET_OK;
}

long long iunet_net_packed_bytes(const iunet_net* n) { return n ? n->packed_bytes : 0; }

int iunet_net_load(iunet_net* n, const void* flat_params, void* packed, void* stream) {
  IUNET_REQUIRE(n && flat_params && packed, "net_load: null pointer");
  const float* P = (const float*)flat_params;
  unsigned char* K = (unsigned char*)packed;
  const float eps = 1e-5f, A = n->act_scale;
  for (const ConvOp& op : n->conv) {
    const float* w = P + op.w;
    const float *g = P + op.bn, *be = g + op.co, *mu = be + op.co, *va = mu + op.co;
    float* aux = (float*)(K + op.aux);
    int rc;
    if (n->mode == 3 && !op.first) {
      float* whi = (float*)(K + n->scratch_off);
      IUNET_CHECK_HIP(hipMemsetAsync(K + op.pk[0], 0, (size_t)iunet_x2m_w8_bytes_nd(n->dim, op.co, op.ci), (hipStream_t)stream));
      rc = iunet_x2m_prep_nd(n->dim, w, whi, K + op.pk[0], aux, aux + op.co, g, be, mu, va, eps, A, A, op.co, op.ci, stream);
      if (rc) return rc;
      rc = iunet_pack_conv3(0, whi, nullptr, K + op.pk[1], op.co, op.ci, n->taps, n->dim == 3 ? 2 : 6, stream);
      if (rc) return rc;
    } else if (n->mode >= 2) {
      float* wv = (float*)(K + n->scratch_off);
      const bool gn = n->norm == 1;
      rc = iunet_x2_prep(w, wv, aux, aux + op.co, gn ? nullptr : g, gn ? nullptr : be, gn ? nullptr : mu, gn ? nullptr : va, nullptr, eps, A, A,
                         op.co, op.ci, n->taps, 0, op.first ? op.ci : (n->dim == 3 ? 16 : 32), stream);
      if (rc) return rc;
      rc = op.first ? iunet_pack_first_conv(0, wv, nullptr, K + op.pk[1], op.co, 3 * op.ci, n->taps, stream)
                    : iunet_pack_conv3(0, wv, nullptr, K + op.pk[1], op.co, 3 * op.ci, n->taps, iunet_x2_pack_mode(n->dim), stream);
      if (rc) return rc;
    } else {
      hipLaunchKernelGGL(net_fold_bn_kernel, dim3((op.co + 255) / 256), dim3(256), 0, (hipStream_t)stream, g, be, mu, va, eps, aux,
                         aux + op.co, op.co);
      IUNET_CHECK_HIP(hipGetLastError());
      if (op.first) rc = iunet_pack_first_conv(n->mode, w, aux, K + op.pk[1], op.co, op.ci, n->taps, stream);
      else {
        rc = iunet_pack_conv3(n->mode, w, aux, K + op.pk[1], op.co, op.ci, n->taps, 2, stream);
        if (!rc && op.pk[0] >= 0) rc = iunet_pack_conv3(n->mode, w, aux, K + op.pk[0], op.co, op.ci, n->taps, 0, stream);
        if (!rc && op.pk[3] >= 0) rc = iunet_pack_conv3(n->mode, w, aux, K + op.pk[3], op.co, op.ci, n->taps, 6, stream);
      }
      if (rc) return rc;
    }
  }
  for (const UpOp& u : n->up) {
    float* aux = (float*)(K + u.aux);
    int rc;
    if (n->mode >= 2) {
      float* wv = (float*)(K + n->scratch_off);
      rc = iunet_x2_prep(P + u.w, wv, aux, aux + u.co, nullptr, nullptr, nullptr, nullptr, P + u.b, eps, A, A, u.co, u.ci, n->npos, 2, 0, stream);
      if (!rc) rc = iunet_pack_convT(0, wv, K + u.pk, 2 * u.ci, u.co, n->npos, stream);
    } else {
      rc = iunet_pack_convT(n->mode, P + u.w, K + u.pk, u.ci, u.co, n->npos, stream);
    }
    if (rc) return rc;
  }
  n->flat = P;
  n->packed = K;
  return IUNET_OK;
}

long long iunet_net_workspace_bytes(const iunet_net* n, int N, int D, int H, int W) {
  if (!n || N < 1 || D < 1 || H < 1 || W < 1) return 0;
  const int f = 1 << (n->levels - 1);
  if (H % f || W % f || (n->dim == 3 && D % f) || (n->dim == 2 && D != 1)) return 0;
  return ws_layout(n, N, D, H, W).bytes;
}

int iunet_net_forward(iunet_net* n, const void* x, int in_dtype, const long long* in_strides, int N, int D, int H, int W, void* workspace,
                      void* logits, void* probs, void* cls, const long long* out_strides, float divisor, int accumulate, void* stream) {
  IUNET_REQUIRE(n && x && in_strides && workspace, "net_forward: null pointer");
  IUNET_REQUIRE(n->packed != nullptr, "net_forward: iunet_net_load has not been called");
  IUNET_REQUIRE(iunet_net_workspace_bytes(n, N, D, H, W) > 0, "net_forward: spatial size %d x %d x %d must be divisible by %d (D == 1 in 2-D)",
                D, H, W, 1 << (n->levels - 1));
  IUNET_REQUIRE((logits == nullptr && probs == nullptr) || out_strides != nullptr, "net_forward: logits / probs need out_strides");
  const WsLayout L = ws_layout(n, N, D, H, W);
  unsigned char* WS = (unsigned char*)workspace;
  unsigned char* K = n->packed;
  const int lv = n->levels, dim = n->dim, mode = n->mode;
  if (n->nested) return nested_forward(n, L, x, in_dtype, in_strides, N, D, H, W, WS, logits, probs, cls, out_strides, divisor, accumulate, stream);
  if (mode == 3) {
    const float A = n->act_scale;
    void* sat = WS;
    auto dims3 = [&](int l, int& d, int& h, int& w) { d = dim == 3 ? D >> l : 1; h = H >> l; w = W >> l; };
    auto vox3 = [&](int l) { return (long long)(dim == 3 ? D >> l : 1) * (H >> l) * (W >> l); };
    auto convm = [&](const ConvOp& op, long long xo, long long x_ss, long long x8o, long long x8_ss, long long yo, long long y_ss, int y_lo,
                     long long y8o, long long y8_ss, int l) -> int {
      int d, h, w;
      dims3(l, d, h, w);
      const float* aux = (const float*)(K + op.aux);
      return iunet_x2m_conv_fwd(dim, WS + xo, x_ss, WS + x8o, x8_ss, WS + yo, y_ss, y_lo, y8o >= 0 ? WS + y8o : nullptr, y8_ss, K + op.pk[1], K + op.pk[0],
                                aux, aux + op.co, N, d, h, w, op.ci, op.co, 2, sat, stream);
    };
    int rc = 0;
    for (int l = 0; l < lv; ++l) {
      int d, h, w;
      dims3(l, d, h, w);
      const long long v = vox3(l);
      const int c = n->ch[l];
      const ConvOp& c1 = n->conv[2 * stage_index(n, false, l)];
      const ConvOp& c2 = n->conv[2 * stage_index(n, false, l) + 1];
      if (l == 0 && lv > 1 && iunet_x2m_first_stage_fusable(dim, n->cin, c, N, h, w)) {
        const float* aux1 = (const float*)(K + c1.aux);
        const float* aux2 = (const float*)(K + c2.aux);
        const bool pooled = iunet_x2m_pool_fusable(dim, c) != 0;
        rc = iunet_x2m_first_stage_fwd(x, in_dtype, in_strides, K + c1.pk[1], aux1, aux1 + c, A, WS + L.cat[0], 2ll * c * v, -1, WS + L.catm[0], 2ll * c * v,
                                       pooled ? WS + L.pin[1] : nullptr, (long long)c * vox3(1), pooled ? WS + L.pinm[1] : nullptr, (long long)c * vox3(1),
                                       K + c2.pk[1], K + c2.pk[0], aux2, aux2 + c2.co, N, h, w, sat, stream);
        if (rc) return rc;
        if (!pooled) {
          int dn, hn, wn;
          dims3(1, dn, hn, wn);
          rc = iunet_x2m_maxpool_fwd(dim, WS + L.cat[0], 2ll * c * v, WS + L.catm[0], 2ll * c * v, WS + L.pin[1], (long long)c * vox3(1), WS + L.pinm[1],
                                     (long long)c * vox3(1), c, N, dn, hn, wn, stream);
          if (rc) return rc;
        }
        continue;
      }
      if (l == 0) {
        const float* aux = (const float*)(K + c1.aux);
        rc = iunet_x2m_first_conv_fwd(dim, x, in_dtype, in_strides, WS + L.a[0], (long long)c * v, -1, WS + L.am[0], (long long)c * v, K + c1.pk[1], aux,
                                      aux + c, A, N, d, h, w, n->cin, c, 1, sat, stream);
      } else {
        const int cp = n->ch[l - 1];
        rc = convm(c1, L.pin[l], (long long)cp * v, L.pinm[l], (long long)cp * v, L.a[l], (long long)c * v, -1, L.am[l], (long long)c * v, l);
      }
      if (rc) return rc;
      if (l < lv - 1) {
        if (iunet_x2m_pool_fusable(dim, c)) {
          const float* aux = (const float*)(K + c2.aux);
          rc = iunet_x2m_conv_pool_fwd(dim, WS + L.a[l], (long long)c * v, WS + L.am[l], (long long)c * v, WS + L.cat[l], 2ll * c * v, -1, WS + L.catm[l],
                                       2ll * c * v, WS + L.pin[l + 1], (long long)c * vox3(l + 1), WS + L.pinm[l + 1], (long long)c * vox3(l + 1),
                                       K + c2.pk[1], K + c2.pk[0], aux, aux + c2.co, N, d, h, w, c2.ci, c2.co, 2, sat, stream);
        } else {
          rc = convm(c2, L.a[l], (long long)c * v, L.am[l], (long long)c * v, L.cat[l], 2ll * c * v, -1, L.catm[l], 2ll * c * v, l);
          if (rc) return rc;
          int dn, hn, wn;
          dims3(l + 1, dn, hn, wn);
          rc = iunet_x2m_maxpool_fwd(dim, WS + L.cat[l], 2ll * c * v, WS + L.catm[l], 2ll * c * v, WS + L.pin[l + 1], (long long)c * vox3(l + 1),
                                     WS + L.pinm[l + 1], (long long)c * vox3(l + 1), c, N, dn, hn, wn, stream);
        }
      } else {
        rc = convm(c2, L.a[l], (long long)c * v, L.am[l], (long long)c * v, L.b[l], 2ll * c * v, c / 8, -1, 0, l);
      }
      if (rc) return rc;
    }
    for (int l = lv - 2; l >= 0; --l) {
      int di, hi, wi;
      dims3(l + 1, di, hi, wi);
      const long long v = vox3(l), vi = vox3(l + 1);
      const int c = n->ch[l], cn = n->ch[l + 1];
      const UpOp& u = n->up[lv - 2 - l];
      const float* aux = (const float*)(K + u.aux);
      rc = iunet_x2m_convT_fwd(dim, WS + L.b[l + 1], 2ll * cn * vi, cn / 8, WS + L.cat[l] + (long long)(c / 8) * v * 16, 2ll * c * v, -1,
                               WS + L.catm[l] + (long long)(c / 16) * v * 16, 2ll * c * v, K + u.pk, aux, aux + c, N, di, hi, wi, cn, c, sat, stream);
      if (rc) return rc;
      const ConvOp& c1 = n->conv[2 * stage_index(n, true, l)];
      const ConvOp& c2 = n->conv[2 * stage_index(n, true, l) + 1];
      rc = convm(c1, L.cat[l], 2ll * c * v, L.catm[l], 2ll * c * v, L.a[l], (long long)c * v, -1, L.am[l], (long long)c * v, l);
      if (rc) return rc;
      if (l == 0 && (logits || probs || cls) && iunet_x2m_head_fusable(n->ncls, c)) {
        const long long dflt0[5] = {n->ncls * v, v, (long long)H * W, W, 1};
        const float* aux2 = (const float*)(K + c2.aux);
        return iunet_x2m_conv_head_fwd(dim, WS + L.a[0], (long long)c * v, WS + L.am[0], (long long)c * v, K + c2.pk[1], K + c2.pk[0], aux2, aux2 + c,
                                       n->flat + n->head_w, n->flat + n->head_b, A, n->ncls, logits, probs, cls, out_strides ? out_strides : dflt0,
                                       divisor, accumulate, N, dim == 3 ? D : 1, H, W, c, sat, stream);
      }
      rc = convm(c2, L.a[l], (long long)c * v, L.am[l], (long long)c * v, L.b[l], 2ll * c * v, c / 8, -1, 0, l);
      if (rc) return rc;
    }
    if (!logits && !probs && !cls) return IUNET_OK;
    const long long v0 = vox3(0);
    const long long dflt[5] = {n->ncls * v0, v0, (long long)H * W, W, 1};
    const int c0 = n->ch[0];
    return iunet_x2_head_fwd(WS + L.b[0], 2ll * c0 * v0, c0 / 8, c0, n->flat + n->head_w, n->flat + n->head_b, A, n->ncls, logits, probs, cls,
                             out_strides ? out_strides : dflt, divisor, accumulate, N, D, H, W, stream);
  }
  const bool x2 = mode == 2;
  const int mul = x2 ? 2 : 1;
  auto dims = [&](int l, int& d, int& h, int& w) { d = dim == 3 ? D >> l : 1; h = H >> l; w = W >> l; };
  auto vox = [&](int l) { int d, h, w; dims(l, d, h, w); return (long long)d * h * w; };
  auto plane = [&](long long base_off, int planes, int l) { return (void*)(WS + base_off + (long long)planes * vox(l) * 16); };
  int rc = 0;
  auto conv = [&](const ConvOp& op, const void* xp, long long x_ss, int x_lo, void* yp, long long y_ss, int y_lo, int l) -> int {
    int d, h, w;
    dims(l, d, h, w);
    const float* aux = (const float*)(K + op.aux);
    if (x2 && n->norm == 1) {
      const long long v = (long long)d * h * w;
      int r = iunet_x2_conv3_fwd_flag(dim, xp, x_ss, x_lo, WS + L.raw, 2ll * op.co * v, op.co / 8, K + op.pk[1], aux, aux + op.co, N, d, h, w, op.ci, op.co, 0, WS, stream);
      if (r) return r;
      return iunet_x2_gn_relu_fwd(WS + L.raw, 2ll * op.co * v, op.co / 8, yp, y_ss, y_lo, n->flat + op.bn, n->flat + op.bn + op.co, n->groups, 1e-5f,
                                  n->act_scale, WS + L.gnslab, WS + L.gnsc, WS + L.gnsh, op.co, N, v, WS, stream);
    }
    if (x2) return iunet_x2_conv3_fwd_flag(dim, xp, x_ss, x_lo, yp, y_ss, y_lo, K + op.pk[1], aux, aux + op.co, N, d, h, w, op.ci, op.co, 2, WS, stream);
    int lay = 1;
    if (op.pk[3] >= 0 && iunet_conv3_compact_ok(dim, N, d, h, w, op.ci, op.co, 0, 0)) lay = 3;
    else {
      lay = iunet_conv3_pick_layout(dim, N, d, h, w, op.ci, op.co);
      if (lay == 0 && op.pk[0] < 0) lay = 1;
    }
    return iunet_conv3_fwd(mode, dim, xp, x_ss, yp, y_ss, K + op.pk[lay == 2 ? 1 : lay], aux + op.co, nullptr, N, d, h, w, op.ci, op.co, 2, lay, stream);
  };
  for (int l = 0; l < lv; ++l) {
    int d, h, w;
    dims(l, d, h, w);
    const long long v = vox(l);
    const int c = n->ch[l], c8 = c / 8;
    const ConvOp& c1 = n->conv[2 * stage_index(n, false, l)];
    const ConvOp& c2 = n->conv[2 * stage_index(n, false, l) + 1];
    if (l == 0) {
      const float* aux = (const float*)(K + c1.aux);
      const bool gn = n->norm == 1;
      rc = x2 ? iunet_x2m_first_conv_fwd(dim, x, in_dtype, in_strides, WS + (gn ? L.raw : L.a[0]), 2ll * c * v, c8, nullptr, 0, K + c1.pk[1], aux, aux + c, n->act_scale,
                                         N, d, h, w, n->cin, c, gn ? 0 : 1, WS, stream)
              : iunet_first_conv_fwd(mode, dim, x, in_dtype, in_strides, WS + L.a[0], (long long)c * v, K + c1.pk[1], aux + c, nullptr,
                                     N, d, h, w, n->cin, c, 1, stream);
      if (!rc && x2 && gn)
        rc = iunet_x2_gn_relu_fwd(WS + L.raw, 2ll * c * v, c8, WS + L.a[0], 2ll * c * v, c8, n->flat + c1.bn, n->flat + c1.bn + c, n->groups, 1e-5f, n->act_scale,
// ... 80 lines not shown
```

### interactive-unet_amd/interactive_unet/_native.py

```python
import ctypes
import os

import torch

_HERE = os.path.dirname(os.path.abspath(__file__))
LIB_PATH = os.environ.get('IUNET_LIB') or os.path.join(os.path.dirname(_HERE), 'lib', 'libiunet.so')

_lib = None

c_void_p, c_int, c_ll, c_float = ctypes.c_void_p, ctypes.c_int, ctypes.c_longlong, ctypes.c_float

_SIGS = {
    'iunet_abi_version': [],
    'iunet_conv3_num_tiles': [c_int] * 5,
    'iunet_conv3_stats_parts': [c_int] * 7,
    'iunet_pack_conv3': [c_int, c_void_p, c_void_p, c_void_p, c_int, c_int, c_int, c_int, c_void_p],
    'iunet_pack_first_conv': [c_int, c_void_p, c_void_p, c_void_p, c_int, c_int, c_int, c_void_p],
    'iunet_pack_convT': [c_int, c_void_p, c_void_p, c_int, c_int, c_int, c_void_p],
    'iunet_pack_batch': [c_void_p, c_int, c_int, c_void_p],
    'iunet_conv3_fwd': [c_int, c_int, c_void_p, c_ll, c_void_p, c_ll, c_void_p, c_void_p, c_void_p,
                        c_int, c_int, c_int, c_int, c_int, c_int, c_int, c_int, c_void_p],
    'iunet_conv3_pick_layout': [c_int] * 7,
    'iunet_conv3_tile_pairs': [c_int] * 7,
    'iunet_conv3_compact_ok': [c_int] * 9,
    'iunet_conv3_fwd_act': [c_int, c_int, c_void_p, c_ll, c_void_p, c_ll, c_void_p, c_void_p, c_void_p, c_void_p, c_void_p,
                            c_int, c_int, c_int, c_int, c_int, c_int, c_int, c_int, c_void_p],
    'iunet_first_conv_fwd': [c_int, c_int, c_void_p, c_int, ctypes.POINTER(c_ll), c_void_p, c_ll, c_void_p, c_void_p,
                             c_void_p, c_int, c_int, c_int, c_int, c_int, c_int, c_int, c_void_p],
    'iunet_maxpool_fwd': [c_int, c_int, c_void_p, c_ll, c_void_p, c_ll, c_int, c_int, c_int, c_int, c_int, c_void_p],
    'iunet_convT_fwd': [c_int, c_int, c_void_p, c_ll, c_void_p, c_ll, c_void_p, c_void_p,
                        c_int, c_int, c_int, c_int, c_int, c_int, c_void_p],
    'iunet_head_fwd': [c_int, c_void_p, c_ll, c_int, c_void_p, c_void_p, c_int, c_void_p, c_void_p, c_void_p,
                       ctypes.POINTER(c_ll), c_float, c_int, c_int, c_int, c_int, c_int, c_void_p],
    'iunet_f32_pack_conv': [c_void_p] * 7 + [c_float, c_int, c_int, c_int, c_int, c_void_p],
    'iunet_f32_conv_fwd': [c_int, c_void_p, c_int, ctypes.POINTER(c_ll), c_void_p, c_ll, c_void_p, c_void_p,
                           c_int, c_int, c_int, c_int, c_int, c_int, c_int, c_int, c_void_p],
    'iunet_f32_maxpool_fwd': [c_int, c_void_p, c_ll, c_void_p, c_ll, c_int, c_int, c_int, c_int, c_int, c_void_p],
    'iunet_f32_head_fwd': [c_void_p, c_ll, c_int, c_void_p, c_void_p, c_int, c_void_p, c_void_p, c_void_p,
                           ctypes.POINTER(c_ll), c_float, c_int, c_int, c_int, c_int, c_int, c_void_p],
    'iunet_f32_bn_stats': [c_void_p, c_ll, c_int, c_int, c_ll, c_float, c_float, c_void_p, c_void_p, c_void_p, c_void_p, c_void_p],
    'iunet_f32_bn_relu_fwd': [c_void_p, c_ll, c_void_p, c_ll, c_void_p, c_void_p, c_void_p, c_void_p, c_int, c_int, c_ll, c_void_p],
    'iunet_f32_bn_relu_bwd': [c_void_p, c_ll, c_void_p, c_ll, c_void_p, c_ll, c_void_p, c_void_p, c_void_p, c_void_p, c_void_p, c_void_p,
                              c_int, c_int, c_ll, c_void_p],
    'iunet_f32_maxpool_bwd': [c_int, c_void_p, c_ll, c_void_p, c_ll, c_void_p, c_ll, c_int, c_int, c_int, c_int, c_int, c_int, c_void_p],
    'iunet_f32_wgrad_splits': [c_int] * 7,
    'iunet_f32_wgrad': [c_int, c_void_p, c_ll, c_void_p, c_ll, c_void_p, c_int, c_int, c_int, c_int, c_int, c_int, c_int, c_void_p],
    'iunet_f32_head_loss_num_parts': [c_int, c_ll],
    'iunet_f32_head_loss_fwd': [c_void_p, c_ll, c_int, c_void_p, c_void_p, c_int, c_void_p, c_void_p, c_int, c_int, c_void_p, c_void_p,
                                c_void_p, c_int, c_ll, c_void_p],
    'iunet_f32_head_loss_bwd': [c_void_p, c_ll, c_int, c_void_p, c_void_p, c_int, c_void_p, c_void_p, c_int, c_void_p, c_void_p, c_ll,
                                c_void_p, c_ll, c_int, c_ll, c_void_p],
    'iunet_f32_channel_sum': [c_void_p, c_ll, c_void_p, c_int, c_int, c_ll, c_void_p],
    'iunet_x2_prep': [c_void_p] * 9 + [c_float, c_float, c_float, c_int, c_int, c_int, c_int, c_int, c_void_p],
    'iunet_x2_first_conv_fwd': [c_int, c_void_p, c_int, ctypes.POINTER(c_ll), c_void_p, c_ll, c_int, c_void_p, c_void_p, c_void_p,
                                c_float, c_int, c_int, c_int, c_int, c_int, c_int, c_int, c_void_p],
    'iunet_x2_conv3_fwd': [c_int, c_void_p, c_ll, c_int, c_void_p, c_ll, c_int, c_void_p, c_void_p, c_void_p,
                           c_int, c_int, c_int, c_int, c_int, c_int, c_int, c_void_p],
    'iunet_x2_maxpool_fwd': [c_int, c_void_p, c_ll, c_int, c_void_p, c_ll, c_int, c_int, c_int, c_int, c_int, c_int, c_void_p],
    'iunet_x2_convT_fwd': [c_int, c_void_p, c_ll, c_int, c_void_p, c_ll, c_int, c_void_p, c_void_p, c_void_p,
                           c_int, c_int, c_int, c_int, c_int, c_int, c_void_p],
    'iunet_x2_head_fwd': [c_void_p, c_ll, c_int, c_int, c_void_p, c_void_p, c_float, c_int, c_void_p, c_void_p, c_void_p,
                          ctypes.POINTER(c_ll), c_float, c_int, c_int, c_int, c_int, c_int, c_void_p],
    'iunet_x2m_prep': [c_void_p] * 9 + [c_float, c_float, c_float, c_int, c_int, c_void_p],
    'iunet_x2m_prep_nd': [c_int] + [c_void_p] * 9 + [c_float, c_float, c_float, c_int, c_int, c_void_p],
    'iunet_x2_prep_batch': [c_void_p, c_int, c_int, c_void_p],
    'iunet_x2m_prep_batch': [c_void_p, c_int, c_int, c_void_p],
    'iunet_x2m_conv_fwd': [c_int, c_void_p, c_ll, c_void_p, c_ll, c_void_p, c_ll, c_int, c_void_p, c_ll, c_void_p, c_void_p, c_void_p, c_void_p,
                           c_int, c_int, c_int, c_int, c_int, c_int, c_int, c_void_p, c_void_p],
    'iunet_x2m_conv_pool_fwd': [c_int, c_void_p, c_ll, c_void_p, c_ll, c_void_p, c_ll, c_int, c_void_p, c_ll, c_void_p, c_ll, c_void_p, c_ll,
                                c_void_p, c_void_p, c_void_p, c_void_p, c_int, c_int, c_int, c_int, c_int, c_int, c_int, c_void_p, c_void_p],
    'iunet_x2m_first_stage_fwd': [c_void_p, c_int, ctypes.POINTER(c_ll), c_void_p, c_void_p, c_void_p, c_float, c_void_p, c_ll, c_int, c_void_p, c_ll,
                                  c_void_p, c_ll, c_void_p, c_ll, c_void_p, c_void_p, c_void_p, c_void_p, c_int, c_int, c_int, c_void_p, c_void_p],
    'iunet_x2m_conv_head_fwd': [c_int, c_void_p, c_ll, c_void_p, c_ll, c_void_p, c_void_p, c_void_p, c_void_p, c_void_p, c_void_p, c_float, c_int,
                                c_void_p, c_void_p, c_void_p, ctypes.POINTER(c_ll), c_float, c_int, c_int, c_int, c_int, c_int, c_int, c_void_p, c_void_p],
    'iunet_x2m_make8': [c_void_p, c_ll, c_int, c_void_p, c_ll, c_int, c_int, c_int, c_int, c_int, c_void_p],
    'iunet_x2m_first_conv_fwd': [c_int, c_void_p, c_int, ctypes.POINTER(c_ll), c_void_p, c_ll, c_int, c_void_p, c_ll, c_void_p, c_void_p, c_void_p,
                                 c_float, c_int, c_int, c_int, c_int, c_int, c_int, c_int, c_void_p, c_void_p],
    'iunet_x2m_convT_fwd': [c_int, c_void_p, c_ll, c_int, c_void_p, c_ll, c_int, c_void_p, c_ll, c_void_p, c_void_p, c_void_p,
                            c_int, c_int, c_int, c_int, c_int, c_int, c_void_p, c_void_p],
    'iunet_x2_conv3_fwd_flag': [c_int, c_void_p, c_ll, c_int, c_void_p, c_ll, c_int, c_void_p, c_void_p, c_void_p,
                                c_int, c_int, c_int, c_int, c_int, c_int, c_int, c_void_p, c_void_p],
    'iunet_x2m_maxpool_fwd': [c_int, c_void_p, c_ll, c_void_p, c_ll, c_void_p, c_ll, c_void_p, c_ll, c_int, c_int, c_int, c_int, c_int, c_void_p],
    'iunet_x2m_conv3_fwd': [c_void_p, c_ll, c_void_p, c_ll, c_void_p, c_ll, c_int, c_void_p, c_ll, c_void_p, c_void_p, c_void_p, c_void_p,
                            c_int, c_int, c_int, c_int, c_int, c_int, c_int, c_void_p, c_void_p],
    'iunet_f32_gn_relu_fwd': [c_void_p, c_ll, c_void_p, c_ll, c_void_p, c_void_p, c_int, c_float, c_void_p, c_void_p, c_void_p, c_int, c_int, c_ll, c_void_p],
    'iunet_x2_gn_relu_fwd': [c_void_p, c_ll, c_int, c_void_p, c_ll, c_int, c_void_p, c_void_p, c_int, c_float, c_float, c_void_p, c_void_p, c_void_p,
                             c_int, c_int, c_ll, c_void_p, c_void_p],
    'iunet_x2m_gn_relu_fwd': [c_void_p, c_ll, c_int, c_void_p, c_ll, c_int, c_void_p, c_ll, c_void_p, c_void_p, c_int, c_float, c_float, c_void_p, c_void_p, c_void_p,
                              c_int, c_int, c_ll, c_void_p, c_void_p],
    'iunet_logit_diff': [c_void_p, c_void_p, c_ll, c_void_p, c_void_p],
    'iunet_net_create': [c_int, c_int, c_int, c_int, c_int, c_int, c_float, ctypes.POINTER(c_void_p)],
    'iunet_net_create_ex': [c_int, c_int, c_int, c_int, c_int, c_int, c_float, c_int, c_int, ctypes.POINTER(c_void_p)],
    'iunet_net_create_nested': [c_int, c_int, c_int, c_int, c_int, c_int, ctypes.POINTER(c_void_p)],
    'iunet_net_num_tensors': [c_void_p],
    'iunet_net_param': [c_void_p, c_int, ctypes.c_char_p, c_int, ctypes.POINTER(c_ll), ctypes.POINTER(c_ll)],
    'iunet_net_load': [c_void_p, c_void_p, c_void_p, c_void_p],
    'iunet_net_forward': [c_void_p, c_void_p, c_int, ctypes.POINTER(c_ll), c_int, c_int, c_int, c_int, c_void_p, c_void_p, c_void_p,
                          c_void_p, ctypes.POINTER(c_ll), c_float, c_int, c_void_p],
    'iunet_net_eval_step': [c_void_p, c_void_p, c_int, ctypes.POINTER(c_ll), c_void_p, c_void_p, c_int, c_int, c_int, c_int, c_int, c_int, c_void_p,
                            c_void_p, c_void_p, c_void_p],
    'iunet_net_forward_argmax': [c_void_p, c_void_p, c_void_p, c_int, c_int, c_int, c_int, c_void_p, c_void_p],
    'iunet_train_state_init': [c_void_p, c_float, c_int, c_void_p],
    'iunet_head_loss_bwd_dev': [c_int, c_void_p, c_ll, c_int, c_void_p, c_void_p, c_int, c_void_p, c_void_p, c_int, c_void_p, c_void_p,
                                c_void_p, c_ll, c_void_p, c_void_p, c_void_p, c_int, c_ll, c_void_p],
    'iunet_head_grad_scatter': [c_void_p, c_void_p, c_void_p, c_int, c_int, c_void_p],
    'iunet_adamw_step_dev': [c_void_p, c_void_p, c_void_p, c_void_p, c_ll, c_float, c_float, c_float, c_float, c_float, c_void_p, c_int, c_float, c_void_p],
    'iunet_train_create': [c_int, c_int, c_int, c_int, c_int, c_int, c_int, ctypes.POINTER(c_void_p)],
    'iunet_train_create_ex': [c_int, c_int, c_int, c_int, c_int, c_int, c_int, c_int, c_int, ctypes.POINTER(c_void_p)],
    'iunet_train_create_nested': [c_int, c_int, c_int, c_int, c_int, c_int, c_int, ctypes.POINTER(c_void_p)],
    'iunet_train_num_tensors': [c_void_p],
    'iunet_train_param': [c_void_p, c_int, ctypes.c_char_p, c_int, ctypes.POINTER(c_ll), ctypes.POINTER(c_ll)],
    'iunet_train_num_bn': [c_void_p],
    'iunet_train_bind': [c_void_p, c_void_p, c_void_p, c_void_p, c_void_p, ctypes.POINTER(c_void_p), c_void_p, c_void_p, c_void_p],
    'iunet_train_repack': [c_void_p, c_void_p],
    'iunet_train_forward_backward': [c_void_p, c_void_p, c_int, ctypes.POINTER(c_ll), c_void_p, c_void_p, c_int, c_int, c_int, c_int, c_int,
                                     c_void_p, c_void_p, c_void_p],
    'iunet_train_forward_backward_hooks': [c_void_p, c_void_p, c_int, ctypes.POINTER(c_ll), c_void_p, c_void_p, c_int, c_int, c_int, c_int, c_int,
                                           c_void_p, c_void_p, c_void_p, c_void_p, c_void_p],
    'iunet_train_update': [c_void_p, c_float, c_float, c_float, c_float, c_float, c_float, c_void_p],
    'iunet_train_step': [c_void_p, c_void_p, c_int, ctypes.POINTER(c_ll), c_void_p, c_void_p, c_int, c_int, c_int, c_int, c_int, c_void_p,
                         c_float, c_float, c_float, c_float, c_float, c_void_p, c_void_p],
    'iunet_f8_pack_conv3': [c_void_p] * 5 + [c_float, c_void_p, c_void_p, c_void_p, c_int, c_int, c_int, c_void_p],
    'iunet_conv3_f8_fwd': [c_int, c_int, c_void_p, c_ll, c_void_p, c_ll, c_void_p, c_void_p, c_void_p,
# ... 61 lines not shown
                               c_void_p, c_void_p, c_void_p, c_void_p, c_void_p, c_void_p, c_void_p, c_int, c_int, c_int,
                               c_int, c_int, c_void_p],
    'iunet_bn_relu_sum_bwd': [c_int, c_int, c_int, ctypes.POINTER(c_void_p), ctypes.POINTER(c_ll), c_void_p, c_ll, c_void_p, c_ll,
                              c_void_p, c_ll, c_void_p, c_void_p, c_void_p, c_void_p, c_void_p, c_void_p, c_void_p, c_void_p,
                              c_void_p, c_int, c_int, c_int, c_int, c_int, c_void_p],
    'iunet_maxpool_bwd': [c_int, c_int, c_void_p, c_ll, c_void_p, c_ll, c_void_p, c_ll, c_int, c_int, c_int, c_int,
                          c_int, c_int, c_void_p],
    'iunet_head_loss_num_parts': [c_int, c_ll],
    'iunet_head_loss_bwd_num_parts': [c_int, c_ll, c_int, c_int],
    'iunet_head_loss_fwd': [c_int, c_void_p, c_ll, c_int, c_void_p, c_void_p, c_int, c_void_p, c_void_p, c_int, c_int,
                            c_void_p, c_void_p, c_void_p, c_int, c_ll, c_void_p],
    'iunet_head_loss_bwd': [c_int, c_void_p, c_ll, c_int, c_void_p, c_void_p, c_int, c_void_p, c_void_p, c_int,
                            c_void_p, c_float, c_void_p, c_ll, c_void_p, c_int, c_ll, c_void_p],
    'iunet_head_loss_fwd_act': [c_int, c_void_p, c_ll, c_int, c_void_p, c_void_p, c_int, c_void_p, c_void_p, c_int, c_int,
                                c_void_p, c_void_p, c_void_p, c_void_p, c_void_p, c_int, c_ll, c_void_p],
    'iunet_head_loss_fwd_act_ps': [c_int, c_void_p, c_ll, c_int, c_void_p, c_void_p, c_int, c_void_p, c_void_p, c_int, c_int,
                                   c_void_p, c_void_p, c_void_p, c_void_p, c_void_p, c_int, c_int, c_ll, c_void_p],
    'iunet_head_gn_bwd': [c_int, c_void_p, c_ll, c_int, c_void_p, c_void_p, c_int, c_void_p, c_void_p, c_int, c_void_p, c_float, c_void_p, c_void_p,
                          c_void_p, c_void_p, c_void_p, c_void_p, c_int, c_void_p, c_void_p, c_void_p, c_ll, c_void_p, c_void_p, c_void_p, c_void_p, c_int, c_ll, c_void_p],
    'iunet_head_loss_bwd_act': [c_int, c_void_p, c_ll, c_int, c_void_p, c_void_p, c_int, c_void_p, c_void_p, c_int,
                                c_void_p, c_float, c_void_p, c_ll, c_void_p, c_void_p, c_void_p, c_int, c_ll, c_void_p],
    'iunet_reduce_slab': [c_void_p, c_int, c_ll, c_void_p, c_float, c_int, c_void_p],
    'iunet_check_finite': [c_void_p, c_ll, c_void_p, c_void_p],
    'iunet_adamw_step': [c_void_p, c_void_p, c_void_p, c_void_p, c_ll, c_float, c_float, c_float, c_float, c_float,
                         c_int, c_float, c_void_p, c_void_p],
    'iunet_conv3_wgrad_blocks': [c_int] * 7,
    'iunet_conv3_wgrad': [c_int, c_int, c_void_p, c_ll, c_void_p, c_ll, c_void_p, c_void_p, c_float,
                          c_int, c_int, c_int, c_int, c_int, c_int, c_void_p],
    'iunet_conv3_wgrad_act': [c_int, c_int, c_void_p, c_ll, c_void_p, c_ll, c_void_p, c_void_p, c_float, c_void_p, c_void_p,
                              c_int, c_int, c_int, c_int, c_int, c_int, c_void_p],
    'iunet_pack_convT_dgrad': [c_int, c_void_p, c_void_p, c_int, c_int, c_int, c_void_p],
    'iunet_convT_dgrad': [c_int, c_int, c_void_p, c_ll, c_void_p, c_ll, c_void_p, c_int, c_int, c_int, c_int, c_int,
                          c_int, c_void_p],
    'iunet_convT_wgrad_blocks': [c_int] * 7,
    'iunet_convT_wgrad': [c_int, c_int, c_void_p, c_ll, c_void_p, c_ll, c_void_p, c_void_p, c_void_p, c_void_p,
                          c_int, c_int, c_int, c_int, c_int, c_int, c_void_p],
    'iunet_first_conv_wgrad_blocks': [c_int] * 5,
    'iunet_first_conv_wgrad_bn': [c_int, c_int, c_void_p, c_int, ctypes.POINTER(c_ll), c_void_p, c_ll, c_void_p, c_ll, c_void_p,
                                  c_void_p, c_void_p, c_void_p, c_void_p, c_void_p, c_void_p, c_int, c_int, c_int, c_int, c_int,
                                  c_int, c_void_p],
    'iunet_first_conv_wgrad': [c_int, c_int, c_void_p, c_int, ctypes.POINTER(c_ll), c_void_p, c_ll, c_void_p, c_void_p,
                               c_int, c_int, c_int, c_int, c_int, c_int, c_void_p],
    'iunet_lk_pack': [c_int, c_int, c_int] + [c_void_p] * 5 + [c_float, c_void_p, c_void_p, c_int, c_int, c_void_p],
    'iunet_lk_stats_parts': [c_int] * 7,
    'iunet_lk_conv_fwd': [c_int, c_int, c_int, c_void_p, c_ll, c_void_p, c_ll, c_void_p, c_void_p, c_void_p, c_void_p, c_void_p, c_ll,
                          c_void_p, c_int, c_int, c_int, c_int, c_int, c_int, c_int, c_void_p],
    'iunet_lk_wgrad': [c_int, c_int, c_int, c_void_p, c_ll, c_void_p, c_ll, c_void_p, c_void_p, c_void_p, c_void_p, c_float,
                       c_int, c_int, c_int, c_int, c_int, c_int, c_void_p],
    'iunet_lk_bn_relu_add': [c_int, c_void_p, c_ll, c_void_p, c_ll, c_void_p, c_ll, c_void_p, c_void_p, c_int, c_int, c_ll, c_void_p],
    'iunet_lk_f32_conv_fwd': [c_int, c_int, c_void_p, c_ll, c_void_p, c_ll, c_void_p, c_void_p, c_void_p, c_ll,
                              c_int, c_int, c_int, c_int, c_int, c_int, c_void_p],
}
_INT_RETURN = ['iunet_pack_desc_bytes', 'iunet_augment_desc_bytes', 'iunet_x2_prep_desc_bytes']
_INT_RETURN_ARGS = {'iunet_zoom_nearest_len': [c_int, ctypes.c_double], 'iunet_x2_convT_kc': [c_int], 'iunet_x2m_head_fusable': [c_int, c_int], 'iunet_x2m_pool_fusable': [c_int, c_int], 'iunet_x2m_first_stage_fusable': [c_int] * 6, 'iunet_x2_pack_mode': [c_int], 'iunet_f8_pack_order': [c_int, c_int]}
_LL_RETURN = {'iunet_gn_precise_slab_bytes': [c_int, c_int, c_ll], 'iunet_net_eval_scratch_bytes': [c_void_p, c_int, c_int, c_int, c_int], 'iunet_x2m_w8_bytes': [c_int] * 2, 'iunet_x2m_w8_bytes_nd': [c_int] * 3, 'iunet_train_num_params': [c_void_p], 'iunet_train_packed_bytes': [c_void_p], 'iunet_train_workspace_bytes': [c_void_p, c_int, c_int, c_int, c_int], 'iunet_conv3_wgrad_slab_floats': [c_int] * 7, 'iunet_f32_pack_conv_elems': [c_int] * 3, 'iunet_f8_pack_conv3_bytes': [c_int] * 3, 'iunet_conv3_f8_workspace_elems': [c_int] * 7, 'iunet_pack_conv3_elems': [c_int] * 4,
              'iunet_pack_first_conv_elems': [c_int] * 3, 'iunet_slice_scatter_workspace_bytes': [c_int],
              'iunet_lk_pack_elems': [c_int] * 4, 'iunet_lk_wgrad_slab_floats': [c_int] * 8,
              'iunet_net_num_params': [c_void_p], 'iunet_net_packed_bytes': [c_void_p], 'iunet_net_workspace_bytes': [c_void_p] + [c_int] * 4}


class NativeError(RuntimeError):
    pass


def lib():
    global _lib
    if _lib is None:
        if not os.path.isfile(LIB_PATH):
            raise NativeError(f'{LIB_PATH} is missing: build it with __graft_entry__.build() '
                              f'(interactive-unet_amd/csrc/build.sh); there is no CPU fallback')
        l = ctypes.CDLL(LIB_PATH)
        l.iunet_last_error.restype = ctypes.c_char_p
        l.iunet_last_error.argtypes = []
        for name, args in _SIGS.items():
            fn = getattr(l, name)
            fn.argtypes = args
            fn.restype = c_int
        for name in _INT_RETURN:
            getattr(l, name).restype = c_int
            getattr(l, name).argtypes = []
        for name, args in _INT_RETURN_ARGS.items():
            getattr(l, name).restype = c_int
            getattr(l, name).argtypes = args
        for name, args in _LL_RETURN.items():
            fn = getattr(l, name)
            fn.argtypes = args
            fn.restype = c_ll
        l.iunet_net_destroy.argtypes, l.iunet_net_destroy.restype = [c_void_p], None
        l.iunet_train_destroy.argtypes, l.iunet_train_destroy.restype = [c_void_p], None
        _lib = l
    return _lib


def exported_symbols():
    return ['iunet_last_error', 'iunet_net_destroy', 'iunet_train_destroy'] + list(_SIGS) + list(_LL_RETURN) + list(_INT_RETURN) + list(_INT_RETURN_ARGS)


def check(status):
    if status != 0:
        raise NativeError(f'libiunet error {status}: {lib().iunet_last_error().decode()}')


def call(name, *args):
    check(getattr(lib(), name)(*args))


def pack_conv3_elems(cout, cin, taps, mode=0):
# ... 127 lines not shown
```

### interactive-unet_amd/interactive_unet/engine_x2.py

```python
import ctypes
import os

import torch

from . import _native as nv
from .engine import BN_EPS, _vox


class EngineX2:
    act_dtype = 'fp16x2'
    weight_dtype = None

    def __init__(self, dim=2, levels=4, base=32, cin=1, ncls=2, device='cuda', act_scale=64.0, mixed=None, norm='batch', groups=8):
        if norm not in ('batch', 'group'):
            raise ValueError("norm must be 'batch' or 'group'")
        if norm == 'group' and base % groups:
            raise ValueError(f'{groups} groups do not divide {base} channels')
        self.norm, self.groups = norm, groups
        if dim not in (2, 3):
            raise ValueError('dim must be 2 or 3')
        if base % 32 != 0:
            raise NotImplementedError('native U-Net needs base channels to be a multiple of 32')
        if not (1 <= cin <= 4):
            raise NotImplementedError('native U-Net supports 1..4 input channels')
# ... 39 lines not shown
        ci = (self.cin if l == 0 else self.ch[l - 1]) if prefix.startswith('enc') else 2 * self.ch[l]
        return ci, self.ch[l]

    def _source(self, params, name):
        t = params[name].detach()
        if t.device == self.device and t.dtype == torch.float32 and t.is_contiguous():
            return t
        st = self._stage.get(name)
        if st is None or st.shape != t.shape:
            st = self._stage[name] = torch.empty(t.shape, dtype=torch.float32, device=self.device)
        st.copy_(t)
        return st

    def load_eval(self, params):
        if not hasattr(self, '_stage'):
            self._stage, self._bufs, self._eval_sig, self._eval_tables = {}, {}, None, None
        self._gparams, self._g_dirty, self._g_fwd = params, True, 0
        self.reset_saturation()
        dev = self.device
        lib, A = nv.lib(), self.act_scale
        src = {}
        for prefix in self.stage_names():
            for j in (1, 2):
                src[f'{prefix}.conv{j}.weight'] = self._source(params, f'{prefix}.conv{j}.weight')
                for k in ('weight', 'bias', 'running_mean', 'running_var'):
                    src[f'{prefix}.bn{j}.{k}'] = self._source(params, f'{prefix}.bn{j}.{k}')
        for l in range(self.levels - 1):
            src[f'dec{l}.up.weight'] = self._source(params, f'dec{l}.up.weight')
            src[f'dec{l}.up.bias'] = self._source(params, f'dec{l}.up.bias')
        src['head.weight'] = self._source(params, 'head.weight')
        src['head.bias'] = self._source(params, 'head.bias')
        sig = tuple(t.data_ptr() for t in src.values())
        if sig != self._eval_sig:
            P, d_x2, d_x2m, d_pack, per_layer = {}, [], [], [], []

            def bufs(name, n_virtual, n_packed, co):
                b = self._bufs.get(name)
                if b is None:
                    b = self._bufs[name] = (torch.empty(n_virtual, dtype=torch.float32, device=dev),
                                            torch.empty(n_packed, dtype=torch.float16, device=dev),
                                            torch.empty(co, dtype=torch.float32, device=dev), torch.empty(co, dtype=torch.float32, device=dev))
                return b
            for prefix in self.stage_names():
                ci, co = self.stage_io(prefix)
                for j, (a, b) in enumerate(((ci, co), (co, co)), 1):
                    name = f'{prefix}.conv{j}'
                    first = prefix == 'enc0' and j == 1
                    w = src[f'{name}.weight']
                    bn = [src[f'{prefix}.bn{j}.{k}'] for k in ('weight', 'bias', 'running_mean', 'running_var')]
                    gn = self.norm == 'group'
                    if self.mixed and not first:
                        key = name + '#m'
                        bm = self._bufs.get(key)
                        pmode = 2 if self.dim == 3 else 6
                        if bm is None:
                            bm = self._bufs[key] = (torch.empty(b * a * self.taps, dtype=torch.float32, device=dev),
                                                    torch.empty(nv.pack_conv3_elems(b, a, self.taps, pmode), dtype=torch.float16, device=dev),
                                                    torch.zeros(lib.iunet_x2m_w8_bytes_nd(self.dim, b, a), dtype=torch.uint8, device=dev),
                                                    torch.empty(b, dtype=torch.float32, device=dev), torch.empty(b, dtype=torch.float32, device=dev))
                        whi, w16, w8, osc, bias = bm
                        d_x2m.append(nv.make_x2_prep_desc(w, whi, osc, bias, b, a, self.taps, 3, 0, A, A, bn=None if gn else bn, w8=w8, eps=BN_EPS))
                        d_pack.append(nv.make_desc(whi, w16, b, a, self.taps, 1 if pmode == 2 else 6, torch.float16))
                        bnq = [None] * 4 if gn else [nv.ptr(t) for t in bn]
                        per_layer.append(('iunet_x2m_prep_nd', (self.dim, nv.ptr(w), nv.ptr(whi), nv.ptr(w8), nv.ptr(osc), nv.ptr(bias), bnq[0],
                                                                bnq[1], bnq[2], bnq[3], BN_EPS, A, A, b, a)))
                        per_layer.append(('iunet_pack_conv3', (0, nv.ptr(whi), None, nv.ptr(w16), b, a, self.taps, pmode)))
                        P[name] = (w16, osc, bias, w8, bn[0], bn[1]) if gn else (w16, osc, bias, w8)
                        continue
                    pmode = lib.iunet_x2_pack_mode(self.dim)
                    npk = lib.iunet_pack_first_conv_elems(b, 3 * a, self.taps) if first else nv.pack_conv3_elems(b, 3 * a, self.taps, pmode)
                    wv, dst, osc, bias = bufs(name, b * 3 * a * self.taps, npk, b)
                    kc = a if first else (16 if self.dim == 3 else 32)
                    d_x2.append(nv.make_x2_prep_desc(w, wv, osc, bias, b, a, self.taps, 0, kc, A, A, bn=None if gn else bn, eps=BN_EPS))
                    d_pack.append(nv.make_desc(wv, dst, b, 3 * a, self.taps, 2 if first else (1 if pmode == 2 else 6), torch.float16))
                    bnp = [None] * 4 if gn else [nv.ptr(t) for t in bn]
                    per_layer.append(('iunet_x2_prep', (nv.ptr(w), nv.ptr(wv), nv.ptr(osc), nv.ptr(bias), bnp[0], bnp[1], bnp[2],
                                                        bnp[3], None, BN_EPS, A, A, b, a, self.taps, 0, kc)))
                    if first:
                        per_layer.append(('iunet_pack_first_conv', (0, nv.ptr(wv), None, nv.ptr(dst), b, 3 * a, self.taps)))
                    else:
                        per_layer.append(('iunet_pack_conv3', (0, nv.ptr(wv), None, nv.ptr(dst), b, 3 * a, self.taps, pmode)))
                    P[name] = (dst, osc, bias, bn[0], bn[1]) if gn else (dst, osc, bias)
            for l in range(self.levels - 2, -1, -1):
                name = f'dec{l}.up'
                w, b0 = src[f'{name}.weight'], src[f'{name}.bias']
                ci, co = self.ch[l + 1], self.ch[l]
                wv, dst, osc, bias = bufs(name, 2 * ci * co * self.npos, 2 * ci * co * self.npos, co)
                d_x2.append(nv.make_x2_prep_desc(w, wv, osc, bias, co, ci, self.npos, 2, lib.iunet_x2_convT_kc(ci), A, A, bias_in=b0, eps=BN_EPS))
                d_pack.append(nv.make_desc(wv, dst, co, 2 * ci, self.npos, 3, torch.float16))
                per_layer.append(('iunet_x2_prep', (nv.ptr(w), nv.ptr(wv), nv.ptr(osc), nv.ptr(bias), None, None, None, None, nv.ptr(b0), BN_EPS, A, A,
                                                    co, ci, self.npos, 2, 0)))
                per_layer.append(('iunet_pack_convT', (0, nv.ptr(wv), nv.ptr(dst), 2 * ci, co, self.npos)))
                P[name] = (dst, osc, bias)
            P['head'] = (src['head.weight'].reshape(self.ncls, self.ch[0]), src['head.bias'])
            tabs = [nv.X2PrepTable(d_x2, dev, False)] + ([nv.X2PrepTable(d_x2m, dev, True)] if d_x2m else [])
            tabs.append(nv.PackTable(d_pack, dev, sources=list(src.values())))
            self._eval_tables, self._per_layer, self._eval_sig, self.packed = tabs, per_layer, sig, P
        if os.environ.get('IUNET_X2_PREP_PER_LAYER'):
            s = nv.stream()
            for fn, args in self._per_layer:
                nv.call(fn, *args, s)
            return
        for t in self._eval_tables:
            t.run()

    def level_dims(self, D, H, W):
        return [((D >> l) if self.dim == 3 else 1, H >> l, W >> l) for l in range(self.levels)]
# ... 109 lines not shown
            return self._head(ws, N, D, H, W, logits, probs, cls, out_strides, divisor, accumulate, s)
        for l in range(L):
            d, v = dims[l], _vox(dims[l])
            c8 = ch[l] // 8
            if l == 0:
                w, osc, b = self.packed['enc0.conv1'][:3]
                gn = self.norm == 'group'
                nv.call('iunet_x2m_first_conv_fwd', self.dim, nv.ptr(x), nv.IN_DTYPE_CODE[x.dtype], nv.ll_array(x_strides),
                        Pt(ws['raw'] if gn else ws['a0']), 2 * ch[0] * v, c8, None, 0, nv.ptr(w), nv.ptr(osc), nv.ptr(b), self.act_scale,
                        N, d[0], d[1], d[2], self.cin, ch[0], 0 if gn else 1, nv.ptr(self._sat), s)
                if gn:
                    self._gn('enc0.conv1', ws, Pt(ws['a0']), 2 * ch[0] * v, c8, N, d, ch[0], s)
            else:
                self._conv3(f'enc{l}.conv1', Pt(ws[f'pin{l}']), 2 * ch[l - 1] * v, ch[l - 1] // 8, Pt(ws[f'a{l}']), 2 * ch[l] * v, c8,
                            N, d, ch[l - 1], ch[l], s, ws)
            if l < L - 1:
                self._conv3(f'enc{l}.conv2', Pt(ws[f'a{l}']), 2 * ch[l] * v, c8, Pt(ws[f'cat{l}']), 4 * ch[l] * v, 2 * c8,
                            N, d, ch[l], ch[l], s, ws)
                do = dims[l + 1]
                nv.call('iunet_x2_maxpool_fwd', self.dim, Pt(ws[f'cat{l}']), 4 * ch[l] * v, 2 * c8, Pt(ws[f'pin{l + 1}']),
                        2 * ch[l] * _vox(do), c8, ch[l], N, do[0], do[1], do[2], s)
            else:
                self._conv3(f'enc{l}.conv2', Pt(ws[f'a{l}']), 2 * ch[l] * v, c8, Pt(ws[f'b{l}']), 2 * ch[l] * v, c8,
                            N, d, ch[l], ch[l], s, ws)
        for l in range(L - 2, -1, -1):
            d, v, di, vi = dims[l], _vox(dims[l]), dims[l + 1], _vox(dims[l + 1])
            c8 = ch[l] // 8
            w, osc, b = self.packed[f'dec{l}.up']
            nv.call('iunet_x2m_convT_fwd', self.dim, Pt(ws[f'b{l + 1}']), 2 * ch[l + 1] * vi, ch[l + 1] // 8,
                    Pt(ws[f'cat{l}'], c8, v), 4 * ch[l] * v, 2 * c8, None, 0, nv.ptr(w), nv.ptr(osc), nv.ptr(b),
                    N, di[0], di[1], di[2], ch[l + 1], ch[l], nv.ptr(self._sat), s)
            self._conv3(f'dec{l}.conv1', Pt(ws[f'cat{l}']), 4 * ch[l] * v, 2 * c8, Pt(ws[f'a{l}']), 2 * ch[l] * v, c8,
                        N, d, 2 * ch[l], ch[l], s, ws)
            self._conv3(f'dec{l}.conv2', Pt(ws[f'a{l}']), 2 * ch[l] * v, c8, Pt(ws[f'b{l}']), 2 * ch[l] * v, c8,
                        N, d, ch[l], ch[l], s, ws)
        if features_only:
            return ws['b0']
        self._head(ws, N, D, H, W, logits, probs, cls, out_strides, divisor, accumulate, s)

    def _head(self, ws, N, D, H, W, logits, probs, cls, out_strides, divisor, accumulate, s):
        dims, ch = ws['dims'], self.ch
        hw, hb = self.packed['head']
        if out_strides is None:
            v = _vox(dims[0])
            out_strides = (self.ncls * v, v, H * W, W, 1)
        nv.call('iunet_x2_head_fwd', nv.ptr(ws['b0']), 2 * ch[0] * _vox(dims[0]), ch[0] // 8, ch[0], nv.ptr(hw), nv.ptr(hb),
                self.act_scale, self.ncls, nv.ptr(logits), nv.ptr(probs), nv.ptr(cls), nv.ll_array(out_strides),
                float(divisor), int(bool(accumulate)), N, D, H, W, s)

    def _conv3m(self, name, xp, x_ss, x8p, x8_ss, yp, y_ss, y_lo, y8p, y8_ss, N, d, ci, co, s, pool=None):
        w16, osc, b, w8 = self.packed[name][:4]
        if self.norm == 'group':
            ws, v = self._gn_ws, _vox(d)
            nv.call('iunet_x2m_conv_fwd', self.dim, xp, x_ss, x8p, x8_ss, nv.ptr(ws['raw']), 2 * co * v, co // 8, None, 0, nv.ptr(w16), nv.ptr(w8),
                    nv.ptr(osc), nv.ptr(b), N, d[0], d[1], d[2], ci, co, 0, nv.ptr(self._sat), s)
            return self._gnm(name, ws, yp, y_ss, y_lo, y8p, y8_ss, N, d, co, s)
        probe = self.probe if (self.probe is not None and self.probe['name'] == name) else None
        if probe is not None:
            e0 = torch.cuda.Event(enable_timing=True)
            e0.record()
        if pool is not None:
            nv.call('iunet_x2m_conv_pool_fwd', self.dim, xp, x_ss, x8p, x8_ss, yp, y_ss, y_lo, y8p, y8_ss, pool[0], pool[1], pool[2], pool[3],
                    nv.ptr(w16), nv.ptr(w8), nv.ptr(osc), nv.ptr(b), N, d[0], d[1], d[2], ci, co, 2, nv.ptr(self._sat), s)
        else:
            nv.call('iunet_x2m_conv_fwd', self.dim, xp, x_ss, x8p, x8_ss, yp, y_ss, y_lo, y8p, y8_ss, nv.ptr(w16), nv.ptr(w8), nv.ptr(osc), nv.ptr(b),
                    N, d[0], d[1], d[2], ci, co, 2, nv.ptr(self._sat), s)
        if probe is not None:
            e1 = torch.cuda.Event(enable_timing=True)
            e1.record()
            probe['events'].append((e0, e1, N))

    def _infer_mixed(self, ws, x, x_strides, N, D, H, W, s, head=None, views=None, heads=None):
        dims, L, ch = ws['dims'], self.levels, self.ch
        gn = self.norm == 'group'
        self._gn_ws = ws
        if views is None:
            views = [(x, x_strides, N)]
        P8 = lambda t, planes16=0, v=0: ctypes.c_void_p(t.data_ptr() + planes16 * v * 16)
        Ph = lambda t, planes=0, v=0: ctypes.c_void_p(t.data_ptr() + planes * v * 16)
        stage0 = L > 1 and bool(nv.lib().iunet_x2m_first_stage_fusable(self.dim, self.cin, ch[0], N, H, W)) and self.probe is None and len(views) == 1 and not gn
        for l in range(L):
            d, v = dims[l], _vox(dims[l])
            c = ch[l]
            if l == 0 and stage0:
                fw, fosc, fb = self.packed['enc0.conv1']
                w16, osc, b, w8 = self.packed['enc0.conv2']
                do = dims[1]
                pooled = bool(nv.lib().iunet_x2m_pool_fusable(self.dim, c))
                pool = (Ph(ws['pin1']), c * _vox(do), P8(ws['pin1m']), c * _vox(do))
                nv.call('iunet_x2m_first_stage_fwd', nv.ptr(x), nv.IN_DTYPE_CODE[x.dtype], nv.ll_array(x_strides), nv.ptr(fw), nv.ptr(fosc), nv.ptr(fb),
                        self.act_scale, Ph(ws['cat0']), 2 * c * v, -1, P8(ws['cat0m']), 2 * c * v, *(pool if pooled else (None, 0, None, 0)),
                        nv.ptr(w16), nv.ptr(w8), nv.ptr(osc), nv.ptr(b), N, d[1], d[2], nv.ptr(self._sat), s)
                if not pooled:
                    nv.call('iunet_x2m_maxpool_fwd', self.dim, Ph(ws['cat0']), 2 * c * v, P8(ws['cat0m']), 2 * c * v,
                            pool[0], pool[1], pool[2], pool[3], c, N, do[0], do[1], do[2], s)
                continue
            if l == 0:
                w, osc, b = self.packed['enc0.conv1'][:3]
                n0 = 0
                for vx, vxs, vn in views:
                    if gn:
                        nv.call('iunet_x2m_first_conv_fwd', self.dim, nv.ptr(vx), nv.IN_DTYPE_CODE[vx.dtype], nv.ll_array(vxs),
                                ctypes.c_void_p(ws['raw'].data_ptr() + n0 * 2 * c * v * 2), 2 * c * v, c // 8, None, 0, nv.ptr(w), nv.ptr(osc), nv.ptr(b),
                                self.act_scale, vn, d[0], d[1], d[2], self.cin, c, 0, nv.ptr(self._sat), s)
                    else:
                        nv.call('iunet_x2m_first_conv_fwd', self.dim, nv.ptr(vx), nv.IN_DTYPE_CODE[vx.dtype], nv.ll_array(vxs),
                                ctypes.c_void_p(ws['a0'].data_ptr() + n0 * c * v * 2), c * v, -1, ctypes.c_void_p(ws['a0m'].data_ptr() + n0 * c * v),
                                c * v, nv.ptr(w), nv.ptr(osc), nv.ptr(b), self.act_scale,
                                vn, d[0], d[1], d[2], self.cin, c, 1, nv.ptr(self._sat), s)
                    n0 += vn
                if gn:
                    self._gnm('enc0.conv1', ws, Ph(ws['a0']), c * v, -1, P8(ws['a0m']), c * v, N, d, c, s)
            else:
                cp = ch[l - 1]
                self._conv3m(f'enc{l}.conv1', Ph(ws[f'pin{l}']), cp * v, P8(ws[f'pin{l}m']), cp * v, Ph(ws[f'a{l}']), c * v, -1,
                             P8(ws[f'a{l}m']), c * v, N, d, cp, c, s)
            if l < L - 1:
                do = dims[l + 1]
                fused = not gn and bool(nv.lib().iunet_x2m_pool_fusable(self.dim, c))
                pool = (Ph(ws[f'pin{l + 1}']), c * _vox(do), P8(ws[f'pin{l + 1}m']), c * _vox(do))
                self._conv3m(f'enc{l}.conv2', Ph(ws[f'a{l}']), c * v, P8(ws[f'a{l}m']), c * v, Ph(ws[f'cat{l}']), 2 * c * v, -1,
                             P8(ws[f'cat{l}m']), 2 * c * v, N, d, c, c, s, pool=pool if fused else None)
                if not fused:
                    nv.call('iunet_x2m_maxpool_fwd', self.dim, Ph(ws[f'cat{l}']), 2 * c * v, P8(ws[f'cat{l}m']), 2 * c * v,
                            pool[0], pool[1], pool[2], pool[3], c, N, do[0], do[1], do[2], s)
            else:
                self._conv3m(f'enc{l}.conv2', Ph(ws[f'a{l}']), c * v, P8(ws[f'a{l}m']), c * v, nv.ptr(ws[f'b{l}']), 2 * c * v, c // 8,
                             None, 0, N, d, c, c, s)
        for l in range(L - 2, -1, -1):
            d, v, di, vi = dims[l], _vox(dims[l]), dims[l + 1], _vox(dims[l + 1])
            c, cn = ch[l], ch[l + 1]
            w, osc, b = self.packed[f'dec{l}.up']
            nv.call('iunet_x2m_convT_fwd', self.dim, nv.ptr(ws[f'b{l + 1}']), 2 * cn * vi, cn // 8, Ph(ws[f'cat{l}'], c // 8, v), 2 * c * v, -1,
                    P8(ws[f'cat{l}m'], c // 16, v), 2 * c * v, nv.ptr(w), nv.ptr(osc), nv.ptr(b), N, di[0], di[1], di[2], cn, c, nv.ptr(self._sat), s)
            self._conv3m(f'dec{l}.conv1', Ph(ws[f'cat{l}']), 2 * c * v, P8(ws[f'cat{l}m']), 2 * c * v, Ph(ws[f'a{l}']), c * v, -1,
                         P8(ws[f'a{l}m']), c * v, N, d, 2 * c, c, s)
            if l == 0 and (head is not None or heads is not None):
                w16, osc, b, w8 = self.packed['dec0.conv2']
                hw, hb = self.packed['head']
                hl = [dict(zip(('logits', 'probs', 'cls', 'out_strides', 'divisor', 'accumulate'), head))] if heads is None else heads
                n0 = 0
                for (_, _, vn), o in zip(views, hl):
                    out_strides = o.get('out_strides') or (self.ncls * v, v, H * W, W, 1)
                    nv.call('iunet_x2m_conv_head_fwd', self.dim, ctypes.c_void_p(ws['a0'].data_ptr() + n0 * c * v * 2), c * v,
                            ctypes.c_void_p(ws['a0m'].data_ptr() + n0 * c * v), c * v, nv.ptr(w16), nv.ptr(w8), nv.ptr(osc),
                            nv.ptr(b), nv.ptr(hw), nv.ptr(hb), self.act_scale, self.ncls, nv.ptr(o.get('logits')), nv.ptr(o.get('probs')),
                            nv.ptr(o.get('cls')), nv.ll_array(out_strides), float(o.get('divisor', 1.0)), int(bool(o.get('accumulate', False))),
                            vn, d[0], d[1], d[2], c, nv.ptr(self._sat), s)
                    n0 += vn
                continue
            self._conv3m(f'dec{l}.conv2', Ph(ws[f'a{l}']), c * v, P8(ws[f'a{l}m']), c * v, nv.ptr(ws[f'b{l}']), 2 * c * v, c // 8,
                         None, 0, N, d, c, c, s)

    def max_stored(self):
        if self._g_last is not None:
            self.infer(*self._g_last, features_only=True)
        m = 0.0
        for ws in self._ws_cache.values():
            for k, t in ws.items():
                if k != 'dims' and t.dtype == torch.float16:
                    m = max(m, float(t.abs().max()))
        return m

    def reset_saturation(self):
        self._sat.zero_()
        if self._g is not None:
            self._g.reset_saturation()

    def saturated(self):
        return int(self._sat.item()) >= 0x7bff or (self._g is not None and self._g.saturated())

    def to_split(self, t):
        N, C = t.shape[:2]
        sp = t.shape[2:]
        v = t.float() * self.act_scale
        hi = v.to(torch.float16)
        lo = (v - hi.float()).to(torch.float16)

        def blocked(u):
            u = u.reshape(N, C // 8, 8, *sp)
            return u.permute(0, 1, *range(3, 3 + len(sp)), 2).contiguous()
        return torch.cat([blocked(hi), blocked(lo)], 1).reshape(-1)

    def from_split(self, flat, N, C, sp):
        t = flat.reshape(N, 2, C // 8, *sp, 8).float()
        t = (t[:, 0] + t[:, 1]) / self.act_scale
        return t.permute(0, 1, 2 + len(sp), *range(2, 2 + len(sp))).reshape(N, C, *sp)
```

Measured before the change: 748.9 million.

## Add compact pair-tiled LDS halo layout for 3-D mixed-precision conv kernel

Adds a CPT variant of the 3-D x2m conv kernel that interleaves two channel-chunk halo images in one compact LDS region and loads weights in paired chunks (4+5 combos) using a new pack mode 6. This becomes the default for 3-D through a new pack-mode query. The main loop is unrolled over chunk pairs so weight loads and barriers can be shared and LDS footprint cut. The pool scratch keys are placed in unused parts of the halo region. It adds pack-mode-aware entry points and plumbing through the Python and C engines, with extra template instantiations and new synchronization subtleties.

```diff
diff --git a/include/iunet.h b/include/iunet.h
--- a/include/iunet.h
+++ b/include/iunet.h
@@ -119,6 +119,18 @@
                             const void* oscale, const void* bias, const void* head_w, const void* head_b, float act_scale, int ncls,
                             void* logits, void* probs, void* cls, const long long* out_strides, float divisor, int accumulate, int N, int D,
                             int H, int W, int Cin, void* sat, void* stream);
+int iunet_x2m_pack_mode(int nd);
+int iunet_x2m_conv_fwd_pm(int nd, const void* x, long long x_ss, const void* x8, long long x8_ss, void* y, long long y_ss, int y_lo, void* y8,
+                          long long y8_ss, const void* w16, const void* w8, const void* oscale, const void* bias, int N, int D, int H, int W,
+                          int Cin, int Cout, int epi, void* sat, int pm, void* stream);
+int iunet_x2m_conv_pool_fwd_pm(int nd, const void* x, long long x_ss, const void* x8, long long x8_ss, void* y, long long y_ss, int y_lo, void* y8,
+                               long long y8_ss, void* py, long long py_ss, void* py8, long long py8_ss, const void* w16, const void* w8,
+                               const void* oscale, const void* bias, int N, int D, int H, int W, int Cin, int Cout, int epi, void* sat, int pm,
+                               void* stream);
+int iunet_x2m_conv_head_fwd_pm(int nd, const void* x, long long x_ss, const void* x8, long long x8_ss, const void* w16, const void* w8,
+                               const void* oscale, const void* bias, const void* head_w, const void* head_b, float act_scale, int ncls,
+                               void* logits, void* probs, void* cls, const long long* out_strides, float divisor, int accumulate, int N, int D,
+                               int H, int W, int Cin, void* sat, int pm, void* stream);
 int iunet_x2m_make8(const void* x, long long x_ss, int x_lo, void* x8, long long x8_ss, int C, int N, int D, int H, int W, void* stream);
 int iunet_x2m_first_conv_fwd(int nd, const void* x, int in_dtype, const long long* in_strides, void* y, long long y_sstride, int y_lo,
                              void* y8, long long y8_sstride, const void* w, const void* oscale, const void* bias, float act_scale, int N,
diff --git a/interactive-unet_amd/csrc/conv3_x2m.hip b/interactive-unet_amd/csrc/conv3_x2m.hip
--- a/interactive-unet_amd/csrc/conv3_x2m.hip
+++ b/interactive-unet_amd/csrc/conv3_x2m.hip
@@ -109,7 +109,23 @@
   }
 }
 
-template <bool SMALL, int HEAD = 0, bool POOL = false>
+template <bool SMALL, bool CPT> struct XMHalo {
+  static constexpr int PZ = XMTile<SMALL>::TZ + 2, PY = XMTile<SMALL>::TY + 2, PX = XMTile<SMALL>::TX + 2, NPIX = PZ * PY * PX;
+  static constexpr int PLANE16 = ((NPIX * 16 + 255) / 256) * 256;
+  static constexpr int HEADB = 2 * PY * PX * 16;
+  static constexpr int EO = CPT ? PLANE16 - HEADB : 0;
+  static constexpr int PS = CPT ? NPIX * 16 + PLANE16 - HEADB : PLANE16;
+  static constexpr int A16 = ((EO + PS + PLANE16 + 255) / 256) * 256;
+  static constexpr int POOL1 = EO + PLANE16;
+  static constexpr int PLANE8 = PZ * 192 * 16;
+  static constexpr int lds(int head, bool pool) {
+    return A16 + 5 * 3 * 2 * 1024 + 2 * PLANE8 + F8K_WSTEP + 256 + (head > 0 ? 2048 : 0) + (pool && !CPT ? XMTile<SMALL>::NCW * 2048 : 0);
+  }
+  static_assert(!CPT || (XMTile<SMALL>::NCW / 2 * 2048 <= EO && XMTile<SMALL>::NCW / 2 * 2048 <= PS - PLANE16), "CPT: the pool keys fit the odd image's own part");
+  static_assert(!CPT || NPIX * 16 <= PLANE16, "CPT: plane layout");
+};
+
+template <bool SMALL, int HEAD = 0, bool POOL = false, bool CPT = false>
 __global__ __launch_bounds__((XMTile<SMALL>::NCW * 64 + XM_NLT), 1) void conv3_x2m_kernel(ConvX2MParams p) {
   static_assert(!(POOL && HEAD > 0), "the pooled conv is an encoder conv: no head");
   using TL = XMTile<SMALL>;
@@ -118,9 +134,11 @@
   constexpr int NI = TZ * TY / NCW, NR = NI;
   constexpr int PZ = TZ + 2, PY = TY + 2, PX = TX + 2;
   constexpr int NPIX = PZ * PY * PX;
-  constexpr int PLANE16 = ((NPIX * 16 + 255) / 256) * 256;
-  constexpr int A16 = 2 * PLANE16;
+  using HL = XMHalo<SMALL, CPT>;
+  constexpr int PLANE16 = HL::PLANE16, EO = HL::EO, PS = HL::PS;
+  constexpr int A16 = HL::A16;
   constexpr int NCMB = 5, W16 = NCMB * 3 * 2 * 1024;
+  constexpr int WE = 4 * 3 * 2 * 1024, WPAIR = WE + W16;
   constexpr int ZS = 192;
   constexpr int PLANE8 = PZ * ZS * 16;
   constexpr int A8 = 2 * PLANE8;
@@ -128,6 +146,11 @@
   constexpr int OFF_A16 = 0, OFF_W16 = A16, OFF_A8 = OFF_W16 + W16, OFF_W8 = OFF_A8 + A8, OFF_E = OFF_W8 + W8;
   constexpr int OFF_P = OFF_E + 256;
   static_assert(NI == 4 && NCW * NI == TZ * TY, "a consumer wave owns 4 rows of one z slice");
+  static_assert(NPIX == HL::NPIX && PLANE8 == HL::PLANE8, "XMHalo");
+  auto pool_at = [](int w) -> int {
+    if constexpr (CPT) return OFF_A16 + (w < NCW / 2 ? w * 2048 : HL::POOL1 + (w - NCW / 2) * 2048);
+    else return OFF_P + w * 2048;
+  };
 
   extern __shared__ __attribute__((aligned(256))) unsigned char smem[];
 
@@ -195,7 +218,10 @@
       const int tile = k / nchunk, chunk = k - tile * nchunk;
       int n_img, z0, y0, x0;
       tile_origin(tile, n_img, z0, y0, x0);
-      dma_weights((const unsigned char*)p.w16 + ((long long)cob * nchunk + chunk) * W16, OFF_W16, W16);
+      if constexpr (CPT) dma_weights((const unsigned char*)p.w16 + ((long long)cob * (nchunk >> 1) + (chunk >> 1)) * WPAIR + (chunk & 1) * WE,
+                                     OFF_W16, (chunk & 1) ? W16 : WE);
+      else dma_weights((const unsigned char*)p.w16 + ((long long)cob * nchunk + chunk) * W16, OFF_W16, W16);
+      const int img = (CPT && !(k & 1)) ? EO : 0;
       const f16* xc = (const f16*)p.x + (long long)n_img * p.x_sstride + (long long)chunk * 2 * plane_stride;
 #pragma unroll
       for (int it = 0; it < AIT; ++it) {
@@ -210,7 +236,7 @@
 #pragma unroll
             for (int e = 0; e < 2; ++e)
               dma_piece(ok ? (const unsigned char*)(xc + e * plane_stride + goff) : (const unsigned char*)zero16,
-                        __builtin_amdgcn_readfirstlane(lds0 + OFF_A16 + e * PLANE16 + base * 16));
+                        __builtin_amdgcn_readfirstlane(lds0 + OFF_A16 + img + e * PS + base * 16));
           }
         }
       }
@@ -233,14 +259,15 @@
         }
       }
     };
-    auto make_hi8 = [&]() {
+    auto make_hi8 = [&](int k) {
+      const unsigned char* img = smem + OFF_A16 + ((CPT && !(k & 1)) ? EO : 0);
       f16x8 va[DIT], vb[DIT];
 #pragma unroll
       for (int it = 0; it < DIT; ++it) {
         const int c = dcoord[it];
         const int pix = c >= 0 ? ((c >> 16) * PY + ((c >> 8) & 255)) * PX + (c & 255) : 0;
-        va[it] = *(const f16x8*)(smem + OFF_A16 + pix * 16);
-        vb[it] = *(const f16x8*)(smem + OFF_A16 + PLANE16 + pix * 16);
+        va[it] = *(const f16x8*)(img + pix * 16);
+        vb[it] = *(const f16x8*)(img + PS + pix * 16);
       }
 #pragma unroll
       for (int it = 0; it < DIT; ++it) {
@@ -262,12 +289,14 @@
       pw_dst = nullptr;
       if (lt >= NCW * 32) return;
       const int q = lt & 3, x8 = (lt >> 2) & 7, py = (lt >> 5) & 3, pz = lt >> 7;
-      const unsigned char* a = smem + OFF_P + (((((4 * pz + (py >> 1)) * 2 + (py & 1)) * 8 + x8) * 4 + q) * 32);
-      const unsigned char* b = a + 2 * (2 * 8 * 4 * 32);
+      const int wa = 4 * pz + (py >> 1), rest = ((((py & 1) * 8 + x8) * 4 + q) * 32);
+      const unsigned char* a = smem + pool_at(wa) + rest;
+      const unsigned char* b = smem + pool_at(wa + 2) + rest;
       const u32x4 a0 = *(const u32x4*)a, a1 = *(const u32x4*)(a + 16), b0 = *(const u32x4*)b, b1 = *(const u32x4*)(b + 16);
       unsigned kk[8];
 #pragma unroll
       for (int j = 0; j < 4; ++j) { kk[j] = max(a0[j], b0[j]); kk[4 + j] = max(a1[j], b1[j]); }
+      if constexpr (CPT) asm volatile("s_waitcnt lgkmcnt(0)" ::: "memory");
       int n_img, z0, y0, x0;
       tile_origin(tile, n_img, z0, y0, x0);
       const int Do = p.D >> 1, Ho = p.H >> 1, Wo = p.W >> 1;
@@ -294,15 +323,16 @@
       dma8(k);
 #endif
 #if !defined(X2M_ABLATE_NO_HI8) && !defined(X2M_ABLATE_NO_COPIES)
-      make_hi8();
+      make_hi8(k);
 #endif
       landed();
       lds_barrier();
+      const bool pool_now = POOL && k > 0 && k % nchunk == 0;
+      if constexpr (POOL && CPT) { if (pool_now) pool_words(k / nchunk - 1); }
 #ifndef X2M_ABLATE_NO_COPIES
       if (k + 1 < npairs) dma16(k + 1);
 #endif
-      const bool pool_now = POOL && k > 0 && k % nchunk == 0;
-      if constexpr (POOL) { if (pool_now) pool_words(k / nchunk - 1); }
+      if constexpr (POOL && !CPT) { if (pool_now) pool_words(k / nchunk - 1); }
       landed();
       if constexpr (POOL) { if (pool_now) pool_store(); }
       lds_barrier();
@@ -323,7 +353,8 @@
     const int col = min(2 * c + (q >> 1), 8);
     col_off[c] = ((col / 3) * PY * PX + (col % 3)) * 16;
   }
-  const int rbase16 = (q & 1) * PLANE16 + ((((row_first / TY) * PY + (row_first % TY)) * PX) + l15) * 16;
+  const int rbase16 = (q & 1) * PS + ((((row_first / TY) * PY + (row_first % TY)) * PX) + l15) * 16;
+  const int xoff = (q >> 1) ? 0 : EO;
   int coff[2];
 #pragma unroll
   for (int g = 0; g < 2; ++g) {
@@ -347,9 +378,9 @@
   i32x8 R8f[2][NR + 2], A8f[2][2];
   i64 R8n[NR + 2], A8n[3][2];
 
-  auto load_group = [&](int c, auto BUF) {
+  auto load_group = [&](int c, auto BUF, int img = 0) {
     constexpr int b = decltype(BUF)::value;
-    const unsigned char* ab = smem + OFF_A16 + rbase16;
+    const unsigned char* ab = smem + OFF_A16 + img + rbase16;
     const unsigned char* wl = smem + OFF_W16 + lane * 16;
 #pragma unroll
     for (int r = 0; r < NR + 2; ++r) R16[b][r] = *(const f16x8*)(ab + r * PX * 16 + col_off[c]);
@@ -488,7 +519,7 @@
             kk[j] = max(kk[j], lane_xor1(kk[j]));
           }
           if (!(l15 & 1)) {
-            unsigned char* dst = smem + OFF_P + ((((wave * 2 + (n >> 1)) * 8 + (l15 >> 1)) * 4 + q) * 32);
+            unsigned char* dst = smem + pool_at(wave) + ((((n >> 1) * 8 + (l15 >> 1)) * 4 + q) * 32);
             *(u32x4*)dst = u32x4{kk[0], kk[1], kk[2], kk[3]};
             *(u32x4*)(dst + 16) = u32x4{kk[4], kk[5], kk[6], kk[7]};
           }
@@ -506,6 +537,42 @@
   };
 
   lds_barrier();
+  if constexpr (CPT) {
+    auto fp8_step = [&](int img_next) {
+      load_sub(I1{}); mfma_sub(I0{}, N6{});
+      load_sub(I2{}); mfma_sub(I1{}, N6{});
+      load_sub(I3{}); mfma_sub(I2{}, N12{});
+      load_sub(I4{}); mfma_sub(I3{}, N6{});
+      load_sub(I5{}); mfma_sub(I4{}, N6{});
+      load_sub(I6{}); mfma_sub(I5{}, N12{});
+      lds_barrier();
+      load_group(0, I0{}, img_next);
+      mfma_sub(I6{}, N4{}); mfma_sub(I7{}, N4{}); mfma_sub(I8{}, N4{});
+    };
+    load_group(0, I0{}, EO);
+    __builtin_amdgcn_sched_barrier(0);
+    for (int k = 0; k < npairs; k += 2) {
+      load_group(1, I1{}, EO); group_mfmas(I0{}, true);
+      load_group(2, I0{}, EO); group_mfmas(I1{}, true);
+      load_group(3, I1{}, EO); group_mfmas(I0{}, true);
+      lds_barrier();
+      load_sub(I0{});
+      group_mfmas(I1{}, true);
+      fp8_step(0);
+      load_group(1, I1{}, 0); group_mfmas(I0{}, true);
+      load_group(2, I0{}, 0); group_mfmas(I1{}, true);
+      load_group(3, I1{}, 0); group_mfmas(I0{}, true);
+      load_group(4, I0{}, xoff); group_mfmas(I1{}, true);
+      lds_barrier();
+      load_sub(I0{});
+      group_mfmas(I0{}, true);
+      fp8_step(EO);
+      const int tile = (k + 1) / nchunk;
+      if (k + 1 - tile * nchunk == nchunk - 1) tile_epilogue(tile);
+    }
+    if constexpr (POOL) lds_barrier();
+    return;
+  }
   load_group(0, I0{});
   __builtin_amdgcn_sched_barrier(0);
   for (int k = 0; k < npairs; ++k) {
@@ -1062,19 +1129,18 @@
   return IUNET_OK;
 }
 
-template <bool SMALL, int HEAD = 0, bool POOL = false>
+template <bool SMALL, int HEAD = 0, bool POOL = false, bool CPT = false>
 int launch_x2m(ConvX2MParams p, hipStream_t stream) {
   using TL = XMTile<SMALL>;
-  constexpr int PZ = TL::TZ + 2, NPIX = PZ * 10 * 18;
-  constexpr int PLANE16 = ((NPIX * 16 + 255) / 256) * 256, PLANE8 = PZ * 192 * 16;
-  const int lds = 2 * PLANE16 + 30720 + 2 * PLANE8 + F8K_WSTEP + 256 + (HEAD > 0 ? 2048 : 0) + (POOL ? TL::NCW * 64 * 32 : 0);
-  IUNET_SET_MAX_LDS((conv3_x2m_kernel<SMALL, HEAD, POOL>), lds);
+  constexpr int lds = XMHalo<SMALL, CPT>::lds(HEAD, POOL);
+  static_assert(lds <= 160 * 1024, "conv3_x2m: LDS");
+  IUNET_SET_MAX_LDS((conv3_x2m_kernel<SMALL, HEAD, POOL, CPT>), lds);
   p.tilesZ = (p.D + TL::TZ - 1) / TL::TZ; p.tilesY = (p.H + TL::TY - 1) / TL::TY; p.tilesX = (p.W + TL::TX - 1) / TL::TX;
   const int ncob = p.Cout / 32;
   iunet_brick_shape(3, ncob, p.tilesZ, p.tilesY, p.tilesX, &p.bz, &p.by, &p.bx);
   p.nbz = (p.tilesZ + p.bz - 1) / p.bz; p.nby = (p.tilesY + p.by - 1) / p.by; p.nbx = (p.tilesX + p.bx - 1) / p.bx;
   const int gx = 8 * p.bz * p.by * p.bx;
-  hipLaunchKernelGGL((conv3_x2m_kernel<SMALL, HEAD, POOL>), dim3(gx, ncob), dim3(TL::NCW * 64 + XM_NLT), lds, stream, p);
+  hipLaunchKernelGGL((conv3_x2m_kernel<SMALL, HEAD, POOL, CPT>), dim3(gx, ncob), dim3(TL::NCW * 64 + XM_NLT), lds, stream, p);
   IUNET_CHECK_HIP(hipGetLastError());
   return IUNET_OK;
 }
@@ -1300,10 +1366,16 @@
                         int Cin, int Cout, int epi, void* sat, void* stream) {
   return iunet_x2m_conv_fwd(3, x, x_ss, x8, x8_ss, y, y_ss, y_lo, y8, y8_ss, w16, w8, oscale, bias, N, D, H, W, Cin, Cout, epi, sat, stream);
 }
+int iunet_x2m_pack_mode(int nd) {
+  static const int compact = getenv("IUNET_X2M_COMPACT") ? atoi(getenv("IUNET_X2M_COMPACT")) : 1;
+  IUNET_REQUIRE(nd == 2 || nd == 3, "x2m_pack_mode: nd must be 2 or 3 (got %d)", nd);
+  return nd == 3 && compact == 0 ? 2 : 6;
+}
 static int x2m_conv_impl(const char* who, int nd, const void* x, long long x_ss, const void* x8, long long x8_ss, void* y, long long y_ss, int y_lo,
                          void* y8, long long y8_ss, void* py, long long py_ss, void* py8, long long py8_ss, const void* w16, const void* w8,
-                         const void* oscale, const void* bias, int N, int D, int H, int W, int Cin, int Cout, int epi, void* sat, void* stream) {
+                         const void* oscale, const void* bias, int N, int D, int H, int W, int Cin, int Cout, int epi, void* sat, int pm, void* stream) {
   IUNET_REQUIRE(nd == 2 || nd == 3, "%s: nd must be 2 or 3", who);
+  IUNET_REQUIRE(pm == 6 || (pm == 2 && nd == 3), "%s: the w16 operator's pack mode must be 6%s (got %d)", who, nd == 3 ? " or 2" : "", pm);
   IUNET_REQUIRE(nd == 3 || D == 1, "%s: 2-D needs D == 1", who);
   IUNET_REQUIRE(x && x8 && y && w16 && w8 && oscale, "%s: null pointer", who);
   IUNET_REQUIRE(N > 0 && D > 0 && H > 0 && W > 0, "%s: bad shape N %d, %d x %d x %d", who, N, D, H, W);
@@ -1329,6 +1401,10 @@
   if (nd == 2) return pool ? launch_x2m_2d<0, true>(p, s) : launch_x2m_2d<0>(p, s);
   const long long big_tiles = (long long)N * ((D + 3) / 4) * ((H + 7) / 8) * ((W + 15) / 16);
   const bool small = big_tiles * (Cout / 32) < 128;
+  if (pm == 6) {
+    if (pool) return small ? launch_x2m<true, 0, true, true>(p, s) : launch_x2m<false, 0, true, true>(p, s);
+    return small ? launch_x2m<true, 0, false, true>(p, s) : launch_x2m<false, 0, false, true>(p, s);
+  }
   if (pool) return small ? launch_x2m<true, 0, true>(p, s) : launch_x2m<false, 0, true>(p, s);
   return small ? launch_x2m<true>(p, s) : launch_x2m<false>(p, s);
 }
@@ -1337,7 +1413,13 @@
                        long long y8_ss, const void* w16, const void* w8, const void* oscale, const void* bias, int N, int D, int H, int W,
                        int Cin, int Cout, int epi, void* sat, void* stream) {
   return x2m_conv_impl("x2m_conv3", nd, x, x_ss, x8, x8_ss, y, y_ss, y_lo, y8, y8_ss, nullptr, 0, nullptr, 0, w16, w8, oscale, bias, N, D, H, W,
-                       Cin, Cout, epi, sat, stream);
+                       Cin, Cout, epi, sat, nd == 3 ? 2 : 6, stream);
+}
+int iunet_x2m_conv_fwd_pm(int nd, const void* x, long long x_ss, const void* x8, long long x8_ss, void* y, long long y_ss, int y_lo, void* y8,
+                          long long y8_ss, const void* w16, const void* w8, const void* oscale, const void* bias, int N, int D, int H, int W,
+                          int Cin, int Cout, int epi, void* sat, int pm, void* stream) {
+  return x2m_conv_impl("x2m_conv3", nd, x, x_ss, x8, x8_ss, y, y_ss, y_lo, y8, y8_ss, nullptr, 0, nullptr, 0, w16, w8, oscale, bias, N, D, H, W,
+                       Cin, Cout, epi, sat, pm, stream);
 }
 
 int iunet_x2m_pool_fusable(int nd, int C) {
@@ -1352,7 +1434,15 @@
                             const void* oscale, const void* bias, int N, int D, int H, int W, int Cin, int Cout, int epi, void* sat, void* stream) {
   IUNET_REQUIRE(py && py8, "x2m_conv_pool: null pooled tensor");
   return x2m_conv_impl("x2m_conv_pool", nd, x, x_ss, x8, x8_ss, y, y_ss, y_lo, y8, y8_ss, py, py_ss, py8, py8_ss, w16, w8, oscale, bias, N, D, H, W,
-                       Cin, Cout, epi, sat, stream);
+                       Cin, Cout, epi, sat, nd == 3 ? 2 : 6, stream);
+}
+int iunet_x2m_conv_pool_fwd_pm(int nd, const void* x, long long x_ss, const void* x8, long long x8_ss, void* y, long long y_ss, int y_lo, void* y8,
+                               long long y8_ss, void* py, long long py_ss, void* py8, long long py8_ss, const void* w16, const void* w8,
+                               const void* oscale, const void* bias, int N, int D, int H, int W, int Cin, int Cout, int epi, void* sat, int pm,
+                               void* stream) {
+  IUNET_REQUIRE(py && py8, "x2m_conv_pool: null pooled tensor");
+  return x2m_conv_impl("x2m_conv_pool", nd, x, x_ss, x8, x8_ss, y, y_ss, y_lo, y8, y8_ss, py, py_ss, py8, py8_ss, w16, w8, oscale, bias, N, D, H, W,
+                       Cin, Cout, epi, sat, pm, stream);
 }
 
 int iunet_x2m_first_stage_fusable(int nd, int cin, int c0, int N, int H, int W) {
@@ -1393,11 +1483,23 @@
   return !off && ncls >= 2 && ncls <= 3 && C0 == 32;
 }
 
+int iunet_x2m_conv_head_fwd_pm(int nd, const void* x, long long x_ss, const void* x8, long long x8_ss, const void* w16, const void* w8,
+                               const void* oscale, const void* bias, const void* head_w, const void* head_b, float act_scale, int ncls,
+                               void* logits, void* probs, void* cls, const long long* out_strides, float divisor, int accumulate, int N, int D,
+                               int H, int W, int Cin, void* sat, int pm, void* stream);
 int iunet_x2m_conv_head_fwd(int nd, const void* x, long long x_ss, const void* x8, long long x8_ss, const void* w16, const void* w8,
                             const void* oscale, const void* bias, const void* head_w, const void* head_b, float act_scale, int ncls,
                             void* logits, void* probs, void* cls, const long long* out_strides, float divisor, int accumulate, int N, int D,
                             int H, int W, int Cin, void* sat, void* stream) {
+  return iunet_x2m_conv_head_fwd_pm(nd, x, x_ss, x8, x8_ss, w16, w8, oscale, bias, head_w, head_b, act_scale, ncls, logits, probs, cls, out_strides,
+                                    divisor, accumulate, N, D, H, W, Cin, sat, nd == 3 ? 2 : 6, stream);
+}
+int iunet_x2m_conv_head_fwd_pm(int nd, const void* x, long long x_ss, const void* x8, long long x8_ss, const void* w16, const void* w8,
+                               const void* oscale, const void* bias, const void* head_w, const void* head_b, float act_scale, int ncls,
+                               void* logits, void* probs, void* cls, const long long* out_strides, float divisor, int accumulate, int N, int D,
+                               int H, int W, int Cin, void* sat, int pm, void* stream) {
   IUNET_REQUIRE(nd == 2 || nd == 3, "x2m_conv_head: nd must be 2 or 3");
+  IUNET_REQUIRE(pm == 6 || (pm == 2 && nd == 3), "x2m_conv_head: the w16 operator's pack mode must be 6%s (got %d)", nd == 3 ? " or 2" : "", pm);
   IUNET_REQUIRE(nd == 3 || D == 1, "x2m_conv_head: 2-D needs D == 1");
   IUNET_REQUIRE(x && x8 && w16 && w8 && oscale && bias && head_w && head_b && out_strides, "x2m_conv_head: null pointer");
   IUNET_REQUIRE_GRID("x2m_conv_head", N, D, H, W);
@@ -1420,6 +1522,11 @@
   hipStream_t s = (hipStream_t)stream;
   if (nd == 2) return ncls == 2 ? launch_x2m_2d<2>(p, s) : launch_x2m_2d<3>(p, s);
   const long long big_tiles = (long long)N * ((D + 3) / 4) * ((H + 7) / 8) * ((W + 15) / 16);
+  if (pm == 6) {
+    if (big_tiles < 128)
+      return ncls == 2 ? launch_x2m<true, 2, false, true>(p, s) : launch_x2m<true, 3, false, true>(p, s);
+    return ncls == 2 ? launch_x2m<false, 2, false, true>(p, s) : launch_x2m<false, 3, false, true>(p, s);
+  }
   if (big_tiles < 128)
     return ncls == 2 ? launch_x2m<true, 2>(p, s) : launch_x2m<true, 3>(p, s);
   return ncls == 2 ? launch_x2m<false, 2>(p, s) : launch_x2m<false, 3>(p, s);
diff --git a/interactive-unet_amd/csrc/net.hip b/interactive-unet_amd/csrc/net.hip
--- a/interactive-unet_amd/csrc/net.hip
+++ b/interactive-unet_amd/csrc/net.hip
@@ -19,12 +19,13 @@
 int iunet_x2_head_fwd(const void*, long long, int, int, const void*, const void*, float, int, void*, void*, void*, const long long*, float,
                       int, int, int, int, int, void*);
 int iunet_x2m_prep_nd(int, const void*, void*, void*, void*, void*, const void*, const void*, const void*, const void*, float, float, float, int, int, void*);
-int iunet_x2m_conv_fwd(int, const void*, long long, const void*, long long, void*, long long, int, void*, long long, const void*, const void*,
-                       const void*, const void*, int, int, int, int, int, int, int, void*, void*);
+int iunet_x2m_conv_fwd_pm(int, const void*, long long, const void*, long long, void*, long long, int, void*, long long, const void*, const void*,
+                          const void*, const void*, int, int, int, int, int, int, int, void*, int, void*);
+int iunet_x2m_pack_mode(int);
 long long iunet_x2m_w8_bytes_nd(int, int, int);
 int iunet_x2m_head_fusable(int, int);
-int iunet_x2m_conv_head_fwd(int, const void*, long long, const void*, long long, const void*, const void*, const void*, const void*, const void*,
-                            const void*, float, int, void*, void*, void*, const long long*, float, int, int, int, int, int, int, void*, void*);
+int iunet_x2m_conv_head_fwd_pm(int, const void*, long long, const void*, long long, const void*, const void*, const void*, const void*, const void*,
+                               const void*, float, int, void*, void*, void*, const long long*, float, int, int, int, int, int, int, void*, int, void*);
 int iunet_x2m_first_conv_fwd(int, const void*, int, const long long*, void*, long long, int, void*, long long, const void*, const void*, const void*,
                              float, int, int, int, int, int, int, int, void*, void*);
 int iunet_x2m_convT_fwd(int, const void*, long long, int, void*, long long, int, void*, long long, const void*, const void*, const void*, int, int,
@@ -36,8 +37,8 @@
 int iunet_x2m_first_stage_fusable(int, int, int, int, int, int);
 int iunet_x2m_first_stage_fwd(const void*, int, const long long*, const void*, const void*, const void*, float, void*, long long, int, void*, long long, void*,
                               long long, void*, long long, const void*, const void*, const void*, const void*, int, int, int, void*, void*);
-int iunet_x2m_conv_pool_fwd(int, const void*, long long, const void*, long long, void*, long long, int, void*, long long, void*, long long, void*, long long,
-                            const void*, const void*, const void*, const void*, int, int, int, int, int, int, int, void*, void*);
+int iunet_x2m_conv_pool_fwd_pm(int, const void*, long long, const void*, long long, void*, long long, int, void*, long long, void*, long long, void*,
+                               long long, const void*, const void*, const void*, const void*, int, int, int, int, int, int, int, void*, int, void*);
 int iunet_x2m_conv3_fwd(const void*, long long, const void*, long long, void*, long long, int, void*, long long, const void*, const void*,
                         const void*, const void*, int, int, int, int, int, int, int, void*, void*);
 long long iunet_x2m_w8_bytes(int, int);
@@ -95,6 +96,7 @@
 
 struct iunet_net {
   int dim, levels, base, cin, ncls, mode;
+  int x2m_pm;
   int norm = 0, groups = 8;
   float act_scale;
   int taps, npos;
@@ -269,7 +271,7 @@
   IUNET_REQUIRE(ncls >= 2 && ncls <= 10, "net_create: 2..10 classes (app.py:162; got %d)", ncls);
   IUNET_REQUIRE(mode >= 0 && mode <= 3, "net_create: mode must be 0 (fp16), 1 (bf16), 2 (fp16x2) or 3 (fp16x2, cross terms on fp8), got %d", mode);
   iunet_net* n = new iunet_net();
-  n->dim = dim; n->levels = levels; n->base = base; n->cin = cin; n->ncls = ncls; n->mode = mode;
+  n->dim = dim; n->levels = levels; n->base = base; n->cin = cin; n->ncls = ncls; n->mode = mode; n->x2m_pm = iunet_x2m_pack_mode(dim);
   n->norm = norm; n->groups = groups;
   n->act_scale = act_scale > 0.f ? act_scale : 64.0f;
   n->taps = dim == 3 ? 27 : 9; n->npos = dim == 3 ? 8 : 4;
@@ -289,7 +291,7 @@
       const int vci = (mode == 2 || (mode == 3 && op.first)) ? 3 * op.ci : op.ci;
       if (op.first) op.pk[1] = pk_take(iunet_pack_first_conv_elems(co, vci, n->taps) * 2);
       else if (mode == 3) {
-        op.pk[1] = pk_take(iunet_pack_conv3_elems(co, op.ci, n->taps, dim == 3 ? 2 : 6) * 2);
+        op.pk[1] = pk_take(iunet_pack_conv3_elems(co, op.ci, n->taps, n->x2m_pm) * 2);
         op.pk[0] = pk_take(iunet_x2m_w8_bytes_nd(dim, co, op.ci));
       } else {
         op.pk[1] = pk_take(iunet_pack_conv3_elems(co, vci, n->taps, mode == 2 ? iunet_x2_pack_mode(dim) : 2) * 2);
@@ -373,7 +375,7 @@
       IUNET_CHECK_HIP(hipMemsetAsync(K + op.pk[0], 0, (size_t)iunet_x2m_w8_bytes_nd(n->dim, op.co, op.ci), (hipStream_t)stream));
       rc = iunet_x2m_prep_nd(n->dim, w, whi, K + op.pk[0], aux, aux + op.co, g, be, mu, va, eps, A, A, op.co, op.ci, stream);
       if (rc) return rc;
-      rc = iunet_pack_conv3(0, whi, nullptr, K + op.pk[1], op.co, op.ci, n->taps, n->dim == 3 ? 2 : 6, stream);
+      rc = iunet_pack_conv3(0, whi, nullptr, K + op.pk[1], op.co, op.ci, n->taps, n->x2m_pm, stream);
       if (rc) return rc;
     } else if (n->mode >= 2) {
       float* wv = (float*)(K + n->scratch_off);
@@ -443,8 +445,8 @@
       int d, h, w;
       dims3(l, d, h, w);
       const float* aux = (const float*)(K + op.aux);
-      return iunet_x2m_conv_fwd(dim, WS + xo, x_ss, WS + x8o, x8_ss, WS + yo, y_ss, y_lo, y8o >= 0 ? WS + y8o : nullptr, y8_ss, K + op.pk[1], K + op.pk[0],
-                                aux, aux + op.co, N, d, h, w, op.ci, op.co, 2, sat, stream);
+      return iunet_x2m_conv_fwd_pm(dim, WS + xo, x_ss, WS + x8o, x8_ss, WS + yo, y_ss, y_lo, y8o >= 0 ? WS + y8o : nullptr, y8_ss, K + op.pk[1],
+                                   K + op.pk[0], aux, aux + op.co, N, d, h, w, op.ci, op.co, 2, sat, n->x2m_pm, stream);
     };
     int rc = 0;
     for (int l = 0; l < lv; ++l) {
@@ -483,9 +485,9 @@
       if (l < lv - 1) {
         if (iunet_x2m_pool_fusable(dim, c)) {
           const float* aux = (const float*)(K + c2.aux);
-          rc = iunet_x2m_conv_pool_fwd(dim, WS + L.a[l], (long long)c * v, WS + L.am[l], (long long)c * v, WS + L.cat[l], 2ll * c * v, -1, WS + L.catm[l],
-                                       2ll * c * v, WS + L.pin[l + 1], (long long)c * vox3(l + 1), WS + L.pinm[l + 1], (long long)c * vox3(l + 1),
-                                       K + c2.pk[1], K + c2.pk[0], aux, aux + c2.co, N, d, h, w, c2.ci, c2.co, 2, sat, stream);
+          rc = iunet_x2m_conv_pool_fwd_pm(dim, WS + L.a[l], (long long)c * v, WS + L.am[l], (long long)c * v, WS + L.cat[l], 2ll * c * v, -1, WS + L.catm[l],
+                                          2ll * c * v, WS + L.pin[l + 1], (long long)c * vox3(l + 1), WS + L.pinm[l + 1], (long long)c * vox3(l + 1),
+                                          K + c2.pk[1], K + c2.pk[0], aux, aux + c2.co, N, d, h, w, c2.ci, c2.co, 2, sat, n->x2m_pm, stream);
         } else {
           rc = convm(c2, L.a[l], (long long)c * v, L.am[l], (long long)c * v, L.cat[l], 2ll * c * v, -1, L.catm[l], 2ll * c * v, l);
           if (rc) return rc;
@@ -516,9 +518,9 @@
       if (l == 0 && (logits || probs || cls) && iunet_x2m_head_fusable(n->ncls, c)) {
         const long long dflt0[5] = {n->ncls * v, v, (long long)H * W, W, 1};
         const float* aux2 = (const float*)(K + c2.aux);
-        return iunet_x2m_conv_head_fwd(dim, WS + L.a[0], (long long)c * v, WS + L.am[0], (long long)c * v, K + c2.pk[1], K + c2.pk[0], aux2, aux2 + c,
-                                       n->flat + n->head_w, n->flat + n->head_b, A, n->ncls, logits, probs, cls, out_strides ? out_strides : dflt0,
-                                       divisor, accumulate, N, dim == 3 ? D : 1, H, W, c, sat, stream);
+        return iunet_x2m_conv_head_fwd_pm(dim, WS + L.a[0], (long long)c * v, WS + L.am[0], (long long)c * v, K + c2.pk[1], K + c2.pk[0], aux2, aux2 + c,
+                                          n->flat + n->head_w, n->flat + n->head_b, A, n->ncls, logits, probs, cls, out_strides ? out_strides : dflt0,
+                                          divisor, accumulate, N, dim == 3 ? D : 1, H, W, c, sat, n->x2m_pm, stream);
       }
       rc = convm(c2, L.a[l], (long long)c * v, L.am[l], (long long)c * v, L.b[l], 2ll * c * v, c / 8, -1, 0, l);
       if (rc) return rc;
diff --git a/interactive-unet_amd/interactive_unet/_native.py b/interactive-unet_amd/interactive_unet/_native.py
--- a/interactive-unet_amd/interactive_unet/_native.py
+++ b/interactive-unet_amd/interactive_unet/_native.py
@@ -69,6 +69,13 @@
                            c_int, c_int, c_int, c_int, c_int, c_int, c_int, c_void_p, c_void_p],
     'iunet_x2m_conv_pool_fwd': [c_int, c_void_p, c_ll, c_void_p, c_ll, c_void_p, c_ll, c_int, c_void_p, c_ll, c_void_p, c_ll, c_void_p, c_ll,
                                 c_void_p, c_void_p, c_void_p, c_void_p, c_int, c_int, c_int, c_int, c_int, c_int, c_int, c_void_p, c_void_p],
+    'iunet_x2m_conv_fwd_pm': [c_int, c_void_p, c_ll, c_void_p, c_ll, c_void_p, c_ll, c_int, c_void_p, c_ll, c_void_p, c_void_p, c_void_p, c_void_p,
+                              c_int, c_int, c_int, c_int, c_int, c_int, c_int, c_void_p, c_int, c_void_p],
+    'iunet_x2m_conv_pool_fwd_pm': [c_int, c_void_p, c_ll, c_void_p, c_ll, c_void_p, c_ll, c_int, c_void_p, c_ll, c_void_p, c_ll, c_void_p, c_ll,
+                                   c_void_p, c_void_p, c_void_p, c_void_p, c_int, c_int, c_int, c_int, c_int, c_int, c_int, c_void_p, c_int, c_void_p],
+    'iunet_x2m_conv_head_fwd_pm': [c_int, c_void_p, c_ll, c_void_p, c_ll, c_void_p, c_void_p, c_void_p, c_void_p, c_void_p, c_void_p, c_float, c_int,
+                                   c_void_p, c_void_p, c_void_p, ctypes.POINTER(c_ll), c_float, c_int, c_int, c_int, c_int, c_int, c_int, c_void_p,
+                                   c_int, c_void_p],
     'iunet_x2m_first_stage_fwd': [c_void_p, c_int, ctypes.POINTER(c_ll), c_void_p, c_void_p, c_void_p, c_float, c_void_p, c_ll, c_int, c_void_p, c_ll,
                                   c_void_p, c_ll, c_void_p, c_ll, c_void_p, c_void_p, c_void_p, c_void_p, c_int, c_int, c_int, c_void_p, c_void_p],
     'iunet_x2m_conv_head_fwd': [c_int, c_void_p, c_ll, c_void_p, c_ll, c_void_p, c_void_p, c_void_p, c_void_p, c_void_p, c_void_p, c_float, c_int,
@@ -236,7 +243,7 @@
                               c_int, c_int, c_int, c_int, c_int, c_int, c_void_p],
 }
 _INT_RETURN = ['iunet_pack_desc_bytes', 'iunet_augment_desc_bytes', 'iunet_x2_prep_desc_bytes']
-_INT_RETURN_ARGS = {'iunet_zoom_nearest_len': [c_int, ctypes.c_double], 'iunet_x2_convT_kc': [c_int], 'iunet_x2m_head_fusable': [c_int, c_int], 'iunet_x2m_pool_fusable': [c_int, c_int], 'iunet_x2m_first_stage_fusable': [c_int] * 6, 'iunet_x2_pack_mode': [c_int], 'iunet_f8_pack_order': [c_int, c_int]}
+_INT_RETURN_ARGS = {'iunet_zoom_nearest_len': [c_int, ctypes.c_double], 'iunet_x2_convT_kc': [c_int], 'iunet_x2m_head_fusable': [c_int, c_int], 'iunet_x2m_pool_fusable': [c_int, c_int], 'iunet_x2m_first_stage_fusable': [c_int] * 6, 'iunet_x2_pack_mode': [c_int], 'iunet_x2m_pack_mode': [c_int], 'iunet_f8_pack_order': [c_int, c_int]}
 _LL_RETURN = {'iunet_gn_precise_slab_bytes': [c_int, c_int, c_ll], 'iunet_net_eval_scratch_bytes': [c_void_p, c_int, c_int, c_int, c_int], 'iunet_x2m_w8_bytes': [c_int] * 2, 'iunet_x2m_w8_bytes_nd': [c_int] * 3, 'iunet_train_num_params': [c_void_p], 'iunet_train_packed_bytes': [c_void_p], 'iunet_train_workspace_bytes': [c_void_p, c_int, c_int, c_int, c_int], 'iunet_conv3_wgrad_slab_floats': [c_int] * 7, 'iunet_f32_pack_conv_elems': [c_int] * 3, 'iunet_f8_pack_conv3_bytes': [c_int] * 3, 'iunet_conv3_f8_workspace_elems': [c_int] * 7, 'iunet_pack_conv3_elems': [c_int] * 4,
               'iunet_pack_first_conv_elems': [c_int] * 3, 'iunet_slice_scatter_workspace_bytes': [c_int],
               'iunet_lk_pack_elems': [c_int] * 4, 'iunet_lk_wgrad_slab_floats': [c_int] * 8,
diff --git a/interactive-unet_amd/interactive_unet/engine_x2.py b/interactive-unet_amd/interactive_unet/engine_x2.py
--- a/interactive-unet_amd/interactive_unet/engine_x2.py
+++ b/interactive-unet_amd/interactive_unet/engine_x2.py
@@ -115,7 +115,7 @@
                     if self.mixed and not first:
                         key = name + '#m'
                         bm = self._bufs.get(key)
-                        pmode = 2 if self.dim == 3 else 6
+                        pmode = self._x2m_pm = lib.iunet_x2m_pack_mode(self.dim)
                         if bm is None:
                             bm = self._bufs[key] = (torch.empty(b * a * self.taps, dtype=torch.float32, device=dev),
                                                     torch.empty(nv.pack_conv3_elems(b, a, self.taps, pmode), dtype=torch.float16, device=dev),
@@ -331,19 +331,19 @@
         w16, osc, b, w8 = self.packed[name][:4]
         if self.norm == 'group':
             ws, v = self._gn_ws, _vox(d)
-            nv.call('iunet_x2m_conv_fwd', self.dim, xp, x_ss, x8p, x8_ss, nv.ptr(ws['raw']), 2 * co * v, co // 8, None, 0, nv.ptr(w16), nv.ptr(w8),
-                    nv.ptr(osc), nv.ptr(b), N, d[0], d[1], d[2], ci, co, 0, nv.ptr(self._sat), s)
+            nv.call('iunet_x2m_conv_fwd_pm', self.dim, xp, x_ss, x8p, x8_ss, nv.ptr(ws['raw']), 2 * co * v, co // 8, None, 0, nv.ptr(w16), nv.ptr(w8),
+                    nv.ptr(osc), nv.ptr(b), N, d[0], d[1], d[2], ci, co, 0, nv.ptr(self._sat), self._x2m_pm, s)
             return self._gnm(name, ws, yp, y_ss, y_lo, y8p, y8_ss, N, d, co, s)
         probe = self.probe if (self.probe is not None and self.probe['name'] == name) else None
         if probe is not None:
             e0 = torch.cuda.Event(enable_timing=True)
             e0.record()
         if pool is not None:
-            nv.call('iunet_x2m_conv_pool_fwd', self.dim, xp, x_ss, x8p, x8_ss, yp, y_ss, y_lo, y8p, y8_ss, pool[0], pool[1], pool[2], pool[3],
-                    nv.ptr(w16), nv.ptr(w8), nv.ptr(osc), nv.ptr(b), N, d[0], d[1], d[2], ci, co, 2, nv.ptr(self._sat), s)
+            nv.call('iunet_x2m_conv_pool_fwd_pm', self.dim, xp, x_ss, x8p, x8_ss, yp, y_ss, y_lo, y8p, y8_ss, pool[0], pool[1], pool[2], pool[3],
+                    nv.ptr(w16), nv.ptr(w8), nv.ptr(osc), nv.ptr(b), N, d[0], d[1], d[2], ci, co, 2, nv.ptr(self._sat), self._x2m_pm, s)
         else:
-            nv.call('iunet_x2m_conv_fwd', self.dim, xp, x_ss, x8p, x8_ss, yp, y_ss, y_lo, y8p, y8_ss, nv.ptr(w16), nv.ptr(w8), nv.ptr(osc), nv.ptr(b),
-                    N, d[0], d[1], d[2], ci, co, 2, nv.ptr(self._sat), s)
+            nv.call('iunet_x2m_conv_fwd_pm', self.dim, xp, x_ss, x8p, x8_ss, yp, y_ss, y_lo, y8p, y8_ss, nv.ptr(w16), nv.ptr(w8), nv.ptr(osc), nv.ptr(b),
+                    N, d[0], d[1], d[2], ci, co, 2, nv.ptr(self._sat), self._x2m_pm, s)
         if probe is not None:
             e1 = torch.cuda.Event(enable_timing=True)
             e1.record()
@@ -421,11 +421,11 @@
                 n0 = 0
                 for (_, _, vn), o in zip(views, hl):
                     out_strides = o.get('out_strides') or (self.ncls * v, v, H * W, W, 1)
-                    nv.call('iunet_x2m_conv_head_fwd', self.dim, ctypes.c_void_p(ws['a0'].data_ptr() + n0 * c * v * 2), c * v,
+                    nv.call('iunet_x2m_conv_head_fwd_pm', self.dim, ctypes.c_void_p(ws['a0'].data_ptr() + n0 * c * v * 2), c * v,
                             ctypes.c_void_p(ws['a0m'].data_ptr() + n0 * c * v), c * v, nv.ptr(w16), nv.ptr(w8), nv.ptr(osc),
                             nv.ptr(b), nv.ptr(hw), nv.ptr(hb), self.act_scale, self.ncls, nv.ptr(o.get('logits')), nv.ptr(o.get('probs')),
                             nv.ptr(o.get('cls')), nv.ll_array(out_strides), float(o.get('divisor', 1.0)), int(bool(o.get('accumulate', False))),
-                            vn, d[0], d[1], d[2], c, nv.ptr(self._sat), s)
+                            vn, d[0], d[1], d[2], c, nv.ptr(self._sat), self._x2m_pm, s)
                     n0 += vn
                 continue
             self._conv3m(f'dec{l}.conv2', Ph(ws[f'a{l}']), c * v, P8(ws[f'a{l}m']), c * v, nv.ptr(ws[f'b{l}']), 2 * c * v, c // 8,
```

Result: no change. 751.3 million, median of 6 (+0.3%).
